# alibaba/graph-gpt

Hardware: AMD Instinct MI355X
Metric: graph-tokens/sec (un-padded Eulerian tokens, whole job) + SMTP loss, PCQM4M-v2 base pre-train (higher is better)
Workload: dtype bf16; 1 GPU; pcqm4m-v2-pretrain-base; model=base d768/L12/H12 (122.1M params), per_gpu_batch=256, global_batch=256, seq_len=32, stacked_feat=13, vocab=756, parallelism=dp1, step=fwd+bwd+allreduce+clip+AdamW, reproducible_mode=True

## Files before the change

graph-gpt_amd/_lib.py:

```python
from __future__ import annotations

import contextlib
import ctypes as C
import os

HERE = os.path.dirname(os.path.abspath(__file__))
LIB_PATH = os.environ.get("GGET_LIB_PATH") or os.path.join(HERE, "lib", "libgget_hip.so")

i32, i64, u64, f32, vp, cp = C.c_int32, C.c_int64, C.c_uint64, C.c_float, C.c_void_p, C.c_char_p


class GgetConfig(C.Structure):
    _fields_ = [(n, i32) for n in ("kind", "vocab_size", "hidden_size", "intermediate_size", "num_layers", "num_heads",
                                   "stacked_feat", "next_n_token", "gated_agg", "causal", "max_position", "num_labels",
                                   "score_bias", "pad_token_id")] + \
               [("rms_eps", f32), ("rope_theta", f32), ("layer_scale_init", f32), ("max_tokens", i32), ("max_batch", i32),
                ("path_pdrop", f32), ("mlp_pdrop", f32), ("head_mlp_layers", i32), ("head_mlp", i32 * 4), ("embed_dim", i32)]


class GgetSizes(C.Structure):
    _fields_ = [(n, u64) for n in ("n_params", "param_bf16_bytes", "master_bytes", "adam_bytes", "grad_bf16_bytes",
                                   "workspace_bytes")]


# ... 64 lines not shown
    "gget_debug_set": (i32, [i32, i32]),
    "gget_debug_get": (i32, [i32, C.POINTER(i32)]),
    "gget_debug_occupy": (i32, [vp, u64, i32, i32, i32, vp]),
    "gget_op_gemm_grouped": (i32, [i32, i32, vp, vp, vp, vp, vp, vp, vp, vp, vp, vp]),
    "gget_op_rmsnorm_fwd": (i32, [vp, vp, vp, vp, i32, i32, f32, vp]),
    "gget_op_rmsnorm_bwd": (i32, [vp, vp, vp, vp, vp, vp, vp, i32, i32, vp]),
    "gget_op_embed_fwd": (i32, [vp, vp, vp, vp, i32, i32, i32, i32, vp]),
    "gget_op_embed_bwd": (i32, [vp, vp, vp, vp, vp, vp, i32, i32, i32, i32, i32, i32, vp]),
    "gget_op_qkv_rope": (i32, [vp, vp, vp, vp, vp, vp, i32, i32, i32, vp]),
    "gget_op_smtp2d": (i32, [vp, i32, vp, i32, vp, vp, i32, i32, i32, f32, f32, f32, i32, i32, C.c_uint32, vp]),
    "gget_op_token_sample": (i32, [vp, i32, i32, i32, i32, f32, f32, i32, f32, C.c_uint32, vp, vp, vp]),
    "gget_op_unmask_origin": (i32, [vp, vp, i32, i32, f32, C.c_uint32, i32, vp]),
    "gget_op_unmask_origin_rows": (i32, [vp, vp, i32, i32, vp, C.c_uint32, i32, vp]),
    "gget_op_unmask_ranked": (i32, [vp, vp, vp, i32, i32, i32, vp, i32, vp, vp]),
    "gget_op_gen_plan": (i32, [vp, i32, i32, i32, vp, i32, vp, vp, vp, vp]),
    "gget_op_gen_acc": (i32, [vp, vp, vp, i32, i32, i32, vp, vp]),
    "gget_op_token_confidence": (i32, [vp, i32, i32, i32, i32, vp, vp, vp]),
    "gget_op_smtp_rows": (i32, [vp, vp, vp, vp, vp, i32, i32, i32, C.c_double, C.c_double, C.c_double, C.c_uint32, vp]),
    "gget_op_rope": (i32, [vp, vp, vp, vp, i32, i32, i32, i32, vp]),
    "gget_op_attn_fwd": (i32, [vp, vp, vp, vp, i32, i32, i32, i32, vp, vp, vp, f32, C.c_uint32, vp]),
    "gget_op_attn_bwd": (i32, [vp, vp, vp, vp, vp, vp, vp, i32, i32, i32, i32, vp, vp, vp, f32, C.c_uint32, vp]),
    "gget_op_copy_from_host": (i32, [vp, vp, C.c_uint64, vp]),
    "gget_op_attn_fwd_varlen": (i32, [vp, vp, vp, vp, vp, i32, i32, i32, i32, vp, vp, vp, i32, f32, C.c_uint32, vp]),
    "gget_op_attn_bwd_varlen": (i32, [vp, vp, vp, vp, vp, vp, vp, vp, i32, i32, i32, i32, vp, vp, vp, i32, f32, C.c_uint32, vp]),
    "gget_op_attn_oproj_fwd": (i32, [vp, vp, vp, vp, vp, vp, vp, vp, vp, vp, vp, i32, i32, i32, i32, f32, f32, C.c_uint32, vp, vp]),
    "gget_op_pack_wo": (i32, [vp, C.c_uint64, vp, vp, i32, i32, vp]),
    "gget_op_attn_oproj_bwd": (i32, [vp, vp, vp, vp, vp, vp, vp, i32, C.c_uint64, vp, vp, vp, vp, vp, vp, i32, i32, i32, i32, vp, vp, vp, f32,
                                      C.c_uint32, i32, vp, vp, vp]),
    "gget_op_attn_fwd_ranges": (i32, [vp, vp, vp, vp, vp, i32, i32, i32, i32, f32, C.c_uint32, vp]),
    "gget_op_attn_bwd_ranges": (i32, [vp, vp, vp, vp, vp, vp, vp, vp, i32, i32, i32, i32, f32, C.c_uint32, vp]),
    "gget_op_ranges_from_mask3d": (i32, [vp, vp, vp, i32, i32, vp]),
    "gget_op_attn_bwd_fused": (i32, [vp, vp, vp, vp, vp, vp, vp, vp, vp, vp, i32, i32, i32, i32, f32, C.c_uint32, vp]),
    "gget_set_dropout": (i32, [vp, f32, f32, C.c_uint32]),
    "gget_set_auc": (i32, [vp, i32, C.c_uint32]),
    "gget_set_token_count": (i32, [vp, C.c_int64]),
    "gget_set_option": (i32, [vp, i32, i32]),
    "gget_set_dp_menu": (i32, [vp, i32, i32]),
    "gget_varlen_status": (i32, [vp, vp, vp]),
    "gget_position_status": (i32, [vp, vp, vp]),
    "gget_deferred_status": (i32, [vp, vp, vp]),
    "gget_set_focal_gamma": (i32, [vp, f32]),
    "gget_set_stack_method": (i32, [vp, i32]),
    "gget_set_rope_range": (i32, [vp, f32]),
    "gget_set_raw_embeds": (i32, [vp, vp, i32]),
    "gget_debug_probe": (i32, [vp, i32, C.POINTER(f32)]),
    "gget_debug_gemm_probe": (i32, [i32, C.POINTER(C.c_double), C.POINTER(C.c_double), C.POINTER(i32), C.POINTER(i32)]),
    "gget_set_dropout_ex": (i32, [vp, f32, f32, f32]),
    "gget_op_gateup_geglu": (i32, [vp, vp, vp, vp, i32, i32, i32, vp]),
    "gget_op_down_dgrad_geglu": (i32, [vp, vp, vp, vp, vp, i32, i32, i32, vp]),
    "gget_op_geglu_fwd": (i32, [vp, vp, i32, i32, vp]),
    "gget_op_geglu_bwd": (i32, [vp, vp, vp, i32, i32, vp]),
    "gget_op_ce_fwd_bwd": (i32, [vp, i32, vp, vp, vp, i32, i32, vp, vp, f32, i32, vp]),
    "gget_op_rmsnorm_bwd_copies": (i32, [vp, vp, vp, vp, vp, vp, vp, i32, i32, i32, u64, vp]),
    "gget_op_rmsnorm_dw": (i32, [vp, vp, vp, vp, i32, i32, i32, u64, vp]),
    "gget_op_ls_rmsnorm_fwd": (i32, [vp, vp, vp, vp, vp, vp, vp, i32, i32, f32, vp]),
    "gget_op_accum_layout": (i32, [i32, C.POINTER(i32), C.POINTER(u64)]),
    "gget_op_rmsnorm_bwd_ls": (i32, [vp, vp, vp, vp, vp, vp, vp, vp, vp, vp, vp, i32, i32, vp]),
    "gget_op_rope_table": (i32, [vp, vp, i32, f32, vp]),
    "gget_op_rope_range_table": (i32, [vp, vp, vp, vp, i32, i32, f32, f32, vp]),
    "gget_op_clamp_positions": (i32, [vp, vp, vp, i64, i32, vp]),
    "gget_op_embed_long_ratio": (i32, [vp, vp, i32, i32, i32, i32, vp]),
    "gget_op_ce_full": (i32, [vp, i32, vp, vp, vp, i32, vp, i32, i32, vp, vp, f32, i32, vp, f32, vp, i32, vp]),
    "gget_op_score_fwd": (i32, [vp, vp, vp, vp, vp, vp, i32, i32, i32, vp]),
    "gget_op_score_bwd": (i32, [vp, vp, vp, vp, vp, vp, vp, i32, i32, i32, vp]),
    "gget_op_tok_score_fwd": (i32, [vp, vp, vp, vp, i32, i32, i32, vp]),
    "gget_op_tok_intra_fwd": (i32, [vp, vp, vp, vp, i32, i32, i32, vp]),
    "gget_op_tok_intra_bwd": (i32, [vp, vp, vp, vp, vp, vp, i32, i32, i32, vp]),
    "gget_set_cls_idx": (i32, [vp, vp]),
    "gget_op_tok_ce": (i32, [vp, vp, vp, vp, vp, i32, i32, vp, i32, vp]),
    "gget_op_tok_score_bwd": (i32, [vp, vp, vp, vp, vp, vp, vp, i32, i32, i32, vp]),
    "gget_op_task_loss": (i32, [vp, vp, vp, i32, i32, i32, vp, vp, vp]),
    "gget_op_auc_loss": (i32, [vp, vp, i32, i32, i32, C.c_uint32, vp, vp, vp, vp]),
    "gget_op_pool_rows": (i32, [vp, vp, vp, i32, i32, vp]),
    "gget_op_scatter_rows_f32": (i32, [vp, vp, vp, i32, i32, vp]),
    "gget_op_head_linear_fwd": (i32, [vp, vp, vp, vp, vp, vp, i32, i32, i32, i32, vp]),
    "gget_op_head_linear_bwd": (i32, [vp, vp, vp, vp, vp, vp, vp, i32, i32, i32, i32, vp]),
    "gget_op_lengths": (i32, [vp, vp, i32, i32, vp, vp, i32, i32, vp]),
    "gget_op_sum_lengths": (i32, [vp, i32, vp, vp]),
    "gget_op_varlen_plan": (i32, [vp, i32, i32, vp, vp, vp, vp, vp, vp, vp, vp, vp, vp, i32, i32, i32, i32, i32, vp, vp]),
    "gget_op_rows_to_grid": (i32, [vp, vp, vp, i64, i32, vp]),
    "gget_op_head_compact_ws_bytes": (u64, [i32]),
    "gget_op_head_compact": (i32, [vp, i32, i32, vp, vp, vp, vp, vp, vp, vp, vp, vp, vp, vp]),
    "gget_op_head_slot_sort": (i32, [vp, vp, vp, vp, vp, vp, vp, vp, vp, vp, i32, i32, i64, i32, vp]),
    "gget_op_head_cell_sum": (i32, [vp, vp, vp, vp, vp, vp, i32, i32, i32, vp]),
    "gget_op_gather_rows": (i32, [vp, vp, vp, vp, i32, i32, i32, vp]),
    "gget_op_gather_rows_remap": (i32, [vp, vp, vp, vp, vp, i32, i32, i32, vp, vp]),
    "gget_op_sample_mask_wgt": (i32, [vp, vp, i32, i32, vp]),
    "gget_op_raw_blend": (i32, [vp, vp, i32, i32, vp, vp, vp, i32, i32, vp, i32, vp]),
    "gget_op_raw_tok_grad": (i32, [vp, vp, vp, i32, i32, vp]),
    "gget_op_gemm_indexed": (i32, [i32, vp, vp, vp, i32, i32, i32, i32, i32, i32, vp, vp, vp, i32, vp, vp]),
    "gget_op_rank_metrics_workspace": (C.c_size_t, [i32, i32]),
    "gget_op_rank_metrics": (i32, [vp, i32, vp, i32, i32, i32, vp, vp, vp, vp, vp, vp, C.c_size_t, vp]),
    "gget_op_link_hits_workspace": (C.c_size_t, [i32]),
    "gget_op_link_hits": (i32, [vp, vp, i32, i64, vp, vp, vp, vp, vp, vp, C.c_size_t, vp]),
    "gget_op_link_mrr_workspace": (C.c_size_t, [i32]),
    "gget_op_link_mrr": (i32, [vp, vp, vp, i32, i32, i32, vp, vp, vp, vp, vp, vp, vp, vp, C.c_size_t, vp]),
    "gget_op_cluster_metrics": (i32, [vp, i32, vp, vp, i32, i32, i32, vp, vp, vp, vp]),
}
CLUSTER_MAX_C = 2048

GEMM_NT, GEMM_NN, GEMM_TN = 0, 1, 2
OPT_NORM_FROM_BACKWARD = 1
OPT_SKIP_NONFINITE_STEP = 2
SHARD_CHUNK = 4096
SHARD_PARAMS, SHARD_MASTER, SHARD_ADAM_M, SHARD_ADAM_V, SHARD_SLOTS, SHARD_EMA = 0, 1, 2, 3, 4, 5
TOKENS_AUTO = -2
EPI_NONE, EPI_RESIDUAL, EPI_ATOMIC_F32, EPI_SLAB_F32 = 0, 1, 2, 3

KEY_GEMM_VARIANT, KEY_GEMM_LDS_HEADROOM, KEY_GEMM_SPLIT_LAST, KEY_DETERMINISTIC, KEY_GEMM_STAGGER = 1, 2, 3, 4, 5
KEY_GEMM_ABLATE, KEY_HEAD_DENSE, KEY_HEAD_TILE, KEY_ATTN_OPROJ_OFF, KEY_LS_NORM_BWD_WIDE = 7, 8, 9, 10, 11
KEY_RMS_WIDE, KEY_CE_PARTS, KEY_GEMM_CU_RESERVE, KEY_OCCUPY_FAT, KEY_LINK_GRID, KEY_CE_GENERIC = 13, 14, 15, 16, 18, 19
KEY_EMBED_SORTED = 20
MENU_KEYS = (1, 2, 3, 4, 5, 7, 8, 9, 10, 11, 13, 14, 15, 16, 18, 19, 20)
GEMM_NO_KSPLIT_ND, GEMM_NO_KSPLIT_WGRAD, GEMM_NO_192_ROWS, GEMM_NO_SPLIT_LAST, GEMM_KSPLIT_128_ONLY, GEMM_ONE_BLOCK_PER_CU = 1, 2, 4, 8, 16, 32
GEMM_KSPLIT_DMA8, GEMM_AREA_RULE = 128, 512


def debug_get(key: int) -> int:
    v = i32()
    check(load().gget_debug_get(int(key), C.byref(v)))
    return int(v.value)


@contextlib.contextmanager
def debug_menu(keys):
    saved = {k: debug_get(k) for k in keys}
    try:
        for k, v in keys.items():
            check(load().gget_debug_set(int(k), int(v)))
        yield
    finally:
        for k, v in saved.items():
            check(load().gget_debug_set(k, v))


def gemm_grouped(lib, mode, problems, stream):
    n = len(problems)
    PA, IA = vp * n, i32 * n
    ptr = lambda k: PA(*[p[k].data_ptr() for p in problems])
    num = lambda k: IA(*[int(p[k]) for p in problems])
    return lib.gget_op_gemm_grouped(mode, n, ptr(0), ptr(1), ptr(2), num(3), num(4), num(5), num(6), num(7), num(8), stream)
PROBLEM_SINGLE_LABEL, PROBLEM_REGRESSION_L1, PROBLEM_REGRESSION_MSE, PROBLEM_MULTI_LABEL, PROBLEM_AUC = 0, 1, 2, 3, 4
PROBLEM_TOKEN_CE_INTRA = 6
PROBLEM_TOKEN_CE = 5

_lib = None


class GgetError(RuntimeError):
    pass


def load(path: str = LIB_PATH):
    global _lib
    if _lib is not None:
        return _lib
    import torch
    if not os.path.exists(path):
        raise GgetError(f"{path} is missing: build it with `python graph-gpt_amd/build.py` "
                        "(or __graft_entry__.build()); this engine has no CPU fallback")
    lib = C.CDLL(path)
    for name, (res, args) in SIGNATURES.items():
        fn = getattr(lib, name)
        fn.restype = res
        fn.argtypes = args
    _lib = lib
    return lib


def check(rc: int):
    if rc != 0:
        raise GgetError(f"gget error {rc}: {load().gget_last_error().decode()}")
```

graph-gpt_amd/csrc/engine.hip:

```cpp
#include <dlfcn.h>
#include <stdarg.h>
#include <stdio.h>
#include <string.h>

#include <algorithm>
#include <chrono>
#include <string>
#include <functional>
#include <vector>

#include "common.h"
#include "gemm.h"
#include "kernels.h"
#include <rccl/rccl.h>

static thread_local char g_err[512] = "";
void gget_set_error(const char* fmt, ...) {
  va_list ap;
  va_start(ap, fmt);
  vsnprintf(g_err, sizeof(g_err), fmt, ap);
  va_end(ap);
}
extern "C" const char* gget_last_error(void) { return g_err; }
extern "C" int gget_version(void) { return 101; }
// ... 77 lines not shown
  add_param(pl, "model.embed_tokens.weight", V, d, -1, true, &pl.emb, &pl.emb32);
  if (pl.has_gate) add_param(pl, "stacked_feat_agg.weight", F, d, -1, true, &pl.gate, &pl.gate32);
  if (c.embed_dim > 0) {
    add_param(pl, "embed_layernorm.weight", c.embed_dim, 0, -1, true, &pl.raw_ln, &pl.raw_ln32);
    if (c.kind == GGET_KIND_PRETRAIN) add_param(pl, "emb_mask_token", c.embed_dim, 0, -1, true, &pl.raw_tok, &pl.raw_tok32);
    add_param(pl, "embed_proj.weight", d, c.embed_dim, -1, false, &pl.raw_proj, nullptr);
  }
  pl.layers.resize(L);
  for (int i = 0; i < L; ++i) {
    LayerOff& lo = pl.layers[i];
    const std::string p = "model.layers." + std::to_string(i) + ".";
    add_param(pl, p + "input_layernorm.weight", d, 0, i, true, &lo.ln1, &lo.ln1_32);
    add_param(pl, p + "self_attn.q_proj.weight", d, d, i, false, &lo.wqkv, nullptr);
    add_param(pl, p + "self_attn.k_proj.weight", d, d, i, false, nullptr, nullptr);
    add_param(pl, p + "self_attn.v_proj.weight", d, d, i, false, nullptr, nullptr);
    add_param(pl, p + "self_attn.o_proj.weight", d, d, i, false, &lo.wo, nullptr);
    if (pl.has_ls) add_param(pl, p + "lambda_1", d, 0, i, true, &lo.lam1, &lo.lam1_32);
    add_param(pl, p + "post_attention_layernorm.weight", d, 0, i, true, &lo.ln2, &lo.ln2_32);
    add_param(pl, p + "mlp.gate_proj.weight", ff, d, i, false, &lo.wgu, nullptr);
    add_param(pl, p + "mlp.up_proj.weight", ff, d, i, false, nullptr, nullptr);
    add_param(pl, p + "mlp.down_proj.weight", d, ff, i, false, &lo.wdown, nullptr);
    if (pl.has_ls) add_param(pl, p + "lambda_2", d, 0, i, true, &lo.lam2, &lo.lam2_32);
  }
  add_param(pl, "model.norm.weight", d, 0, (int)L, true, &pl.normf, &pl.normf32);
  if (c.kind == GGET_KIND_PRETRAIN) {
    if (pl.has_ntp) add_param(pl, "n_token_proj.weight", (int64_t)c.next_n_token * d, d, (int)L, false, &pl.ntp, nullptr);
    add_param(pl, "lm_head.weight", V, d, (int)L, false, &pl.lm, nullptr);
    const int64_t Vp = (int64_t)align_up((uint64_t)V, 64);
    pl.lm_pad_off = pl.n_params;
    pl.lm_pad_count = (uint64_t)(Vp - V) * d;
    pl.n_params += align_up(pl.lm_pad_count, 128);
  } else {
    if (c.head_mlp_layers > 0) {
      pl.n_lin = c.head_mlp_layers + 1;
      pl.head_dim[0] = (int)d;
      for (int i = 0; i < c.head_mlp_layers; ++i) pl.head_dim[i + 1] = c.head_mlp[i];
      pl.head_dim[pl.n_lin] = c.num_labels;
      for (int i = 0; i < pl.n_lin; ++i) {
        const std::string p = "score.mlp_modules." + std::to_string(i) + ".";
        add_param(pl, p + "weight", pl.head_dim[i + 1], pl.head_dim[i], (int)L, true, &pl.head_w[i], &pl.head_w32[i]);
        if (c.score_bias) add_param(pl, p + "bias", pl.head_dim[i + 1], 0, (int)L, true, &pl.head_b[i], &pl.head_b32[i]);
      }
    } else {
      add_param(pl, "score.weight", c.num_labels, d, (int)L, true, &pl.score, &pl.score32);
      if (c.score_bias) add_param(pl, "score.bias", c.num_labels, 0, (int)L, true, &pl.sbias, &pl.sbias32);
    }
  }
  return pl;
}

struct Bump {
  uint64_t off = 0;
  uint64_t take(uint64_t bytes) {
    const uint64_t o = off;
    off += align_up(bytes, 256);
    return o;
  }
};

struct LayerWs {
  uint64_t rstd1, xn1, qkv, lse, attn, araw, xmid, rstd2, xn2, gu, h, mraw;
};

struct Ws {
  uint64_t key_len, pool_row, cos_tab, sin_tab, key_lo, key_hi;
  std::vector<uint64_t> xres;
  std::vector<LayerWs> lw;
  uint64_t rstd_f, hidden;
  uint64_t dxa, dxb, dxc, dxn, dqkv, dattn, dgu, dh, delta, dq_acc, dscaled, dscaled2;
  uint64_t scratch32, loss_sum, loss_part, sqnorm, counts, segs, emb_sort, emb_cnt, emb_slab, wg32, lm_slab;
  uint64_t sq_chunks, sq_tiles;
  uint64_t cnt, hc_tot, m_off, l_off, row_idx, sel_src, sel_label, sel_tok, Hm, Pp, Hl, logits, dlogits, dHl, dP, dHm;
  uint64_t ss_tok, ss_cell, ss_l, ss_pos, ss_tile, ss_state, ss_total;
  uint64_t tlogits, tdlogits, pooled_h, auc_lists;
  uint64_t raw_x, raw_xn, raw_rstd, raw_dxn, raw_dx, raw_flag;
  uint64_t rr_cos, rr_sin, rr_ids;
  uint64_t tok_stat;
  uint64_t intra_rs, intra_cls;
  uint64_t long_wgt;
  uint64_t vl_cu, vl_rowb, vl_pos, vl_ids, vl_pad2c, vl_c2p, vl_status;
  uint64_t vl_long;
  uint64_t wo_pack = 0, wot_pack = 0;
  uint64_t pos_safe;
  uint64_t sk_ws;
  uint64_t head_x[6] = {0}, head_a[5] = {0}, head_d[2] = {0};
  uint64_t total;
};

Ws make_ws(const gget_config_t& c, const Plan& pl) {
  Ws w;
  Bump b;
  const uint64_t T = c.max_tokens, d = c.hidden_size, ff = c.intermediate_size, H = c.num_heads, L = c.num_layers;
  const uint64_t Bm = c.max_batch;
  w.key_len = b.take(Bm * 4);
  w.key_lo = b.take(T * 4);
  w.key_hi = b.take(T * 4);
  w.pool_row = b.take(Bm * 4);
  w.cos_tab = b.take((uint64_t)c.max_position * 32 * 4);
  w.sin_tab = b.take((uint64_t)c.max_position * 32 * 4);
  w.xres.resize(L + 1);
  for (uint64_t i = 0; i <= L; ++i) w.xres[i] = b.take(T * d * 2);
  w.lw.resize(L);
  for (uint64_t i = 0; i < L; ++i) {
    LayerWs& l = w.lw[i];
    l.rstd1 = b.take(T * 4);
    l.xn1 = b.take(T * d * 2);
    l.qkv = b.take(T * 3 * d * 2);
    l.lse = b.take(T * H * 4);
    l.attn = b.take(T * d * 2);
    l.araw = pl.has_res ? b.take(T * d * 2) : 0;
    l.xmid = b.take(T * d * 2);
    l.rstd2 = b.take(T * 4);
    l.xn2 = b.take(T * d * 2);
    l.gu = b.take(T * 2 * ff * 2);
    l.h = b.take(T * ff * 2);
    l.mraw = pl.has_res ? b.take(T * d * 2) : 0;
  }
  w.rstd_f = b.take(T * 4);
  w.hidden = b.take(T * d * 2);
  w.dxa = b.take(T * d * 2);
  w.dxb = b.take(T * d * 2);
  w.dxc = b.take(T * d * 2);
  w.dxn = b.take(T * d * 2);
  w.dqkv = b.take(T * 3 * d * 2);
  w.dattn = b.take(T * d * 2);
  w.dgu = b.take(T * 2 * ff * 2);
  w.dh = b.take(T * ff * 2);
  w.delta = b.take(T * H * 4);
  {
    const uint64_t Smax = c.max_tokens / (c.max_batch > 0 ? c.max_batch : 1);
    w.dq_acc = Smax >= 256 ? b.take(((Smax + 255) / 256) * T * d * 2) : 0;
  }
  w.dscaled = pl.has_res ? b.take(T * d * 2) : 0;
  w.dscaled2 = pl.has_res ? b.take(T * d * 2) : 0;
  w.scratch32 = b.take(pl.n_scratch32 * 4);
  w.loss_sum = b.take(256);
  w.loss_part = b.take(2048 * sizeof(float));
  w.sqnorm = b.take(k_grad_sqnorm_ws_bytes());
  w.sq_chunks = b.take(1024 * sizeof(GgetSqChunk));
  w.sq_tiles = b.take((uint64_t)c.num_layers * kSqTilesPerLayer * sizeof(float));
  w.counts = b.take(256);
  w.segs = b.take((uint64_t)pl.params.size() * sizeof(GgetSegment));
  w.wg32 = b.take(kWgSplit * 4 * d * d * 4);
  w.long_wgt = b.take((uint64_t)c.max_batch * 4);
  w.vl_cu = b.take((Bm + 1) * 4);
  w.vl_long = b.take((3 * Bm + 1) * 4);
  w.vl_rowb = b.take(T * 4);
  w.vl_pos = b.take(T * 8);
  w.vl_ids = b.take(T * (uint64_t)c.stacked_feat * 8);
  w.vl_pad2c = b.take(T * 4);
  w.vl_c2p = b.take(T * 4);
  if (d % 64 == 0 && !pl.has_res) {
    w.wo_pack = b.take((uint64_t)c.num_layers * d * d * 2);
    w.wot_pack = b.take((uint64_t)c.num_layers * d * d * 2);
  }
  w.vl_status = b.take(256);
  w.pos_safe = b.take(T * 8);
  w.sk_ws = b.take(gget_gemm_streamk_bytes());
  if (c.embed_dim > 0) {
    const uint64_t e = c.embed_dim;
    w.raw_x = b.take(T * e * 2); w.raw_xn = b.take(T * e * 2); w.raw_rstd = b.take(T * 4);
    w.raw_dxn = b.take(T * e * 2); w.raw_dx = b.take(T * e * 2); w.raw_flag = b.take(T * 4);
  }
  w.rr_cos = b.take(T * 32 * 4);
  w.rr_sin = b.take(T * 32 * 4);
  w.rr_ids = b.take(T * 8);
  w.emb_sort = b.take(k_embed_bwd_ws_elems(T * (uint64_t)c.stacked_feat, (uint64_t)c.vocab_size) * 4);
  w.emb_cnt = k_embed_dense_ok(c.vocab_size, pl.has_gate) ? b.take(T * align_up(c.vocab_size, 64) * 2) : 0;
  w.emb_slab = k_embed_dense_ok(c.vocab_size, pl.has_gate) ? b.take((uint64_t)kEmbDenseSplit * c.vocab_size * d * 4) : 0;
  if (c.kind == GGET_KIND_PRETRAIN) {
    const uint64_t n = c.next_n_token, Vp = align_up(c.vocab_size, 64);
    w.cnt = b.take(T * 4);
    w.hc_tot = b.take(k_head_compact_ws_bytes((int)T));
    w.m_off = b.take(T * 4);
    w.l_off = b.take(T * 4);
    w.row_idx = b.take(T * 4);
    w.sel_src = b.take(T * n * 4);
    w.sel_label = b.take(T * n * 4);
    w.sel_tok = b.take(T * n * 4);
    w.Hm = b.take(T * d * 2);
    w.dHm = b.take(T * d * 2);
    if (n > 1) {
      const uint64_t cap_p = T * n + n * 256;
      w.ss_tok = b.take(cap_p * 4);
      w.ss_cell = b.take(cap_p * 4);
      w.ss_l = b.take(cap_p * 4);
      w.ss_pos = b.take(T * n * 4);
      w.ss_tile = b.take((cap_p / 128 + 1) * 4);
      w.ss_state = b.take(512);
      w.ss_total = b.take(256);
      w.Pp = b.take(cap_p * d * 2);
      w.Hl = b.take(T * n * d * 2);
      w.dHl = b.take(T * n * d * 2);
      w.dP = b.take(T * n * d * 2);
    } else {
      w.Pp = w.Hl = w.Hm;
      w.dHl = w.dP = w.dHm;
    }
    w.lm_slab = b.take((uint64_t)kLmSplit * c.vocab_size * d * 4);
    w.logits = b.take(T * n * Vp * 2);
    w.dlogits = b.take(T * n * Vp * 2);
  } else {
    w.tlogits = b.take(std::max(Bm, T) * c.num_labels * 4);
    w.tdlogits = b.take(std::max(Bm, T) * c.num_labels * 4);
    w.tok_stat = b.take(256);
    w.intra_rs = b.take((Bm + 1) * 4);
    w.intra_cls = b.take(Bm * 8);
    w.auc_lists = b.take(Bm * 2 * 4);
    w.pooled_h = b.take(Bm * d * 2);
    if (pl.n_lin > 0) {
      uint64_t dmax = 0;
      for (int i = 0; i <= pl.n_lin; ++i) dmax = std::max<uint64_t>(dmax, (uint64_t)pl.head_dim[i]);
      w.head_x[0] = w.pooled_h;
      for (int i = 1; i <= pl.n_lin; ++i) w.head_x[i] = b.take(Bm * pl.head_dim[i] * 2);
      for (int i = 0; i < pl.n_lin; ++i) w.head_a[i] = b.take(Bm * pl.head_dim[i] * 2);
      w.head_d[0] = b.take(Bm * dmax * 4);
      w.head_d[1] = b.take(Bm * dmax * 4);
    }
  }
  w.total = b.off;
  return w;
}

int check_cfg(const gget_config_t* c) {
  GGET_REQUIRE(c != nullptr, "null config");
  GGET_REQUIRE(c->hidden_size > 0 && c->hidden_size % 64 == 0, "hidden_size must be a positive multiple of 64");
  GGET_REQUIRE(c->num_heads * 64 == c->hidden_size, "num_heads*64 must equal hidden_size (head_dim is 64)");
  GGET_REQUIRE(c->intermediate_size > 0 && c->intermediate_size % 64 == 0, "intermediate_size must be a multiple of 64");
  GGET_REQUIRE(c->hidden_size <= 2048, "hidden_size > 2048 not supported by the norm kernels");
  GGET_REQUIRE(c->vocab_size > 1 && c->num_layers >= 1 && c->stacked_feat >= 1, "bad vocab/layers/stacked_feat");
  GGET_REQUIRE(c->kind == GGET_KIND_PRETRAIN || c->kind == GGET_KIND_TASK, "bad kind");
  GGET_REQUIRE(c->max_tokens > 0 && c->max_batch > 0 && c->max_position > 0, "bad capacities");
  if (c->kind == GGET_KIND_PRETRAIN) GGET_REQUIRE(c->next_n_token >= 1, "next_n_token must be >= 1");
  else GGET_REQUIRE(c->num_labels >= 1, "num_labels must be >= 1");
  GGET_REQUIRE(c->embed_dim >= 0 && c->embed_dim % 64 == 0 && c->embed_dim <= 2048, "embed_dim must be 0 or a multiple of 64 up to 2048");
  GGET_REQUIRE(c->head_mlp_layers >= 0 && c->head_mlp_layers <= 4, "the MLP score head holds at most 4 hidden layers");
  for (int i = 0; i < c->head_mlp_layers; ++i) GGET_REQUIRE(c->head_mlp[i] > 0, "bad MLP head width");
  return 0;
}

}

static int bucket_of(int layer, int L) { return layer == L ? 0 : layer < 0 ? L + 1 : L - layer; }

static std::vector<std::pair<uint64_t, uint64_t>> bucket_ranges(const gget_config_t& cfg, const Plan& plan) {
  const int L = cfg.num_layers;
  std::vector<std::pair<uint64_t, uint64_t>> r(L + 2, {UINT64_MAX, 0});
  for (const ParamRec& p : plan.params) {
    auto& b = r[bucket_of(p.layer, L)];
    b.first = std::min(b.first, p.off);
    b.second = std::max(b.second, p.off + align_up(p.count, 128));
  }
  if (plan.lm_pad_count) {
    auto& b = r[bucket_of(L, L)];
    b.second = std::max(b.second, plan.lm_pad_off + align_up(plan.lm_pad_count, 128));
  }
// ... 35 lines not shown
    GGET_HIP_CHECK(hipMalloc(&tab, b_it + b_ch + b_cs + b_gs));
    items = reinterpret_cast<const GgetSqChunk*>(tab);
    chunks = items + it.size();
    chunk_slot = reinterpret_cast<const int32_t*>(chunks + ch.size());
    slot_of = chunk_slot + ch_slot.size();
    auto put = [](const void* dst, const void* src, size_t bytes) {
      return bytes ? hipMemcpy(const_cast<void*>(dst), src, bytes, hipMemcpyHostToDevice) : hipSuccess;
    };
    GGET_HIP_CHECK(put(items, it.data(), b_it));
    GGET_HIP_CHECK(put(chunks, ch.data(), b_ch));
    GGET_HIP_CHECK(put(chunk_slot, ch_slot.data(), b_cs));
    GGET_HIP_CHECK(put(slot_of, global_slot.data(), b_gs));
    nitems = (int)it.size();
    nchunks = (int)ch.size();
    nglobal = (int)global_slot.size();
    return 0;
  }
};

struct gget_engine {
  gget_config_t cfg;
  Plan plan;
  Ws ws;
  bf16_t* P;
  float* master;
  float* am;
  float* av;
  float* ema = nullptr;
  float ema_decay_next = -1.f;
  bf16_t* G;
  float* grad_acc = nullptr;
  int grad_acc_count = 0;
  bool grad_from_acc() const { return grad_acc != nullptr && grad_acc_count > 0; }
  const void* grad_src() const { return grad_from_acc() ? (const void*)grad_acc : (const void*)G; }
  unsigned char* W;
  const float* cos_tab;
  const float* sin_tab;
  std::vector<std::pair<uint64_t, uint64_t>> bucket_range;
  std::vector<std::pair<int, int>> bucket_segs;
  int B = 0, S = 0, T = 0, TP = 0;
  bool varlen = false;
  bool wo_packed = false;
  int tc = 0;
  long tc_next = -1;
  bool opt_norm_from_backward = false;
  bool opt_skip_nonfinite = false;
  bool step_needs_norm(float max_grad_norm, const float* gnorm_dev) const { return max_grad_norm > 0.f || gnorm_dev != nullptr || opt_skip_nonfinite; }
  int sq_layers = 0;
  int n_sq_chunks = 0;
  bool emb_cnt_cleared = false;
  bool head_sorted_fwd = false;
  bool tc_from_caller = false;
  int32_t* host_word = nullptr;
  int32_t* host_word_dev = nullptr;
  const int64_t* pos_rows = nullptr;
  const int32_t* row_base() const { return varlen ? wsp<int32_t>(ws.vl_cu) : nullptr; }
  const int32_t* long_list() const { return varlen ? wsp<int32_t>(ws.vl_long) : nullptr; }
  const int64_t* ids = nullptr;
  const int64_t* pos = nullptr;
  const float* sample_wgt = nullptr;
  bool have_labels = false;
  int problem = 0;
  int auc_num_neg = 1;
  const int64_t* cls_idx_next = nullptr;
  float focal_gamma = 0.f;
  bool stack_long = false;
  float rope_range = 0.f;
  const float* raw_next = nullptr;
  bool raw_first_label_only = false;
  bool ls2_done = false;
  bool raw_used = false;
  const float* cos_cur = nullptr;
  const float* sin_cur = nullptr;
  const int64_t* pos_cur = nullptr;
  bool probe = false;
  std::vector<hipEvent_t> probe_ev[2];
  hipEvent_t probe_event(int which, int idx) {
    auto& v = probe_ev[which];
    while ((int)v.size() <= idx) { hipEvent_t e; if (hipEventCreate(&e) != hipSuccess) return nullptr; v.push_back(e); }
    return v[idx];
  }
  std::function<int(hipStream_t)> presync_work;
  bool presync_done = false;
  hipEvent_t count_event = nullptr;
  unsigned auc_seed = 0;
  bool fwd_valid = false;
  float attn_drop_p = 0.f;
  float path_drop_p = 0.f;
  unsigned attn_drop_seed = 0;
  float embed_drop_p = 0.f;
  float mlp_drop_p = 0.f;
  float head_drop_p = 0.f;
  ElemDropArg head_drop() const { return elem_drop(head_drop_p, attn_drop_seed ^ 0x2545F491u); }
  static ElemDropArg elem_drop(float p, unsigned seed, const int32_t* rows = nullptr) {
    if (p <= 0.f) return ElemDropArg{0, 1.f, 0, nullptr};
    return ElemDropArg{(unsigned)(p * 16777216.0f), 1.0f / (1.0f - p), seed, rows};
  }
  const int32_t* drop_rows() const { return varlen ? wsp<int32_t>(ws.vl_c2p) : nullptr; }
  ElemDropArg embed_drop() const { return elem_drop(embed_drop_p, attn_drop_seed ^ 0x5BD1E995u, drop_rows()); }
  ElemDropArg mlp_drop(int layer) const { return elem_drop(mlp_drop_p, attn_drop_seed + 0x7F4A7C15u * (unsigned)(layer + 1), drop_rows()); }
  PathDropArg path_drop(int layer, int which) const {
    const int L = cfg.num_layers;
    const float rate = (path_drop_p > 0.f && L > 1) ? path_drop_p * (float)layer / (float)(L - 1) : 0.f;
    return PathDropArg{rate, attn_drop_seed ^ (0xD6E8FEB8u * (unsigned)(layer * 2 + which + 1)), S, varlen ? wsp<int32_t>(ws.vl_rowb) : nullptr};
  }
  bf16_t* dx_cur = nullptr;
  bool packed = false;
  bool defer_convert = false;
  void* comm = nullptr;
  bool comm_loopback = false;
  int comm_rank = 0, comm_world = 1;
  int dp_reserve_cus = 0;
  bool dp_lds_headroom = false;
  float* comm_f32 = nullptr;
  uint64_t comm_f32_elems = 0;
  int shard_world = 0, shard_rank = 0;
  int shard_slots = 0;
  std::vector<ShardBucket> shard_plan;
  OptWork shard_work;
  int frozen = -1;
  std::vector<std::pair<uint64_t, uint64_t>> train_ranges;
  OptWork frozen_work;
  const OptWork* opt_work(bool sharded) const { return sharded ? &shard_work : frozen >= 0 ? &frozen_work : nullptr; }
  bool truncated() const { return frozen >= 0 && !plan.has_gate && cfg.embed_dim == 0; }
  int first_trainable_layer() const { return frozen < 0 ? 0 : std::min(frozen, cfg.num_layers); }
  std::pair<uint64_t, uint64_t> bucket_train_range(int bucket) const {
    const uint64_t lo = bucket_range[bucket].first, hi = bucket_range[bucket].second;
    if (frozen < 0) return {lo, hi - lo};
    for (const auto& r : train_ranges) {
      const uint64_t a = std::max(lo, r.first), b = std::min(hi, r.first + r.second);
      if (a < b) return {a, b - a};
    }
    return {lo, 0};
  }
  const int32_t* klo() const { return packed ? wsp<int32_t>(ws.key_lo) : nullptr; }
  const int32_t* khi() const { return packed ? wsp<int32_t>(ws.key_hi) : nullptr; }

  template <typename Tp>
  Tp* wsp(uint64_t off) const { return reinterpret_cast<Tp*>(W + off); }
  int bucket_of_layer(int layer) const { return bucket_of(layer, cfg.num_layers); }
};

struct CallScope {
  LaunchMenu m;
  explicit CallScope(gget_engine* h) : m(g_menu) {
    if (h->dp_reserve_cus > 0) {
      m.gemm_cu_reserve = h->dp_reserve_cus;
      m.gemm_lds_headroom = 1;
      m.rms_wide = 0;
    } else if (h->dp_lds_headroom) {
      m.gemm_lds_headroom = 2;
    }
    t_call_menu = &m;
    gget_gemm_streamk_workspace(h->W + h->ws.sk_ws);
  }
  ~CallScope() {
    gget_gemm_streamk_workspace(nullptr);
    t_call_menu = nullptr;
  }
};

extern "C" int gget_query_sizes(const gget_config_t* cfg, gget_sizes_t* out) {
  if (int e = check_cfg(cfg)) return e;
  GGET_REQUIRE(out != nullptr, "null out");
  Plan pl = make_plan(*cfg);
  Ws w = make_ws(*cfg, pl);
// ... 136 lines not shown
  GGET_REQUIRE(embed_p >= 0.f && embed_p < 1.f && mlp_p >= 0.f && mlp_p < 1.f && head_p >= 0.f && head_p < 1.f,
               "dropout probabilities must be in [0, 1)");
  h->head_drop_p = head_p;
  GGET_REQUIRE(mlp_p == 0.f || h->cfg.mlp_pdrop > 0.f, "MLP dropout needs a handle created with config.mlp_pdrop > 0");
  h->embed_drop_p = embed_p;
  h->mlp_drop_p = mlp_p;
  return 0;
}

extern "C" int gget_set_raw_embeds(gget_handle_t h, const float* raw_embeds_dev, int first_label_only) {
  GGET_REQUIRE(h != nullptr, "null handle");
  GGET_REQUIRE(h->cfg.embed_dim > 0 || raw_embeds_dev == nullptr, "the handle was created with embed_dim = 0");
  h->raw_next = raw_embeds_dev;
  h->raw_first_label_only = first_label_only != 0;
  return 0;
}

extern "C" int gget_set_rope_range(gget_handle_t h, float rope_range) {
  GGET_REQUIRE(h != nullptr, "null handle");
  GGET_REQUIRE(rope_range >= 0.f, "rope_range must be >= 0");
  h->rope_range = rope_range;
  return 0;
}

extern "C" int gget_set_stack_method(gget_handle_t h, int stack_long) {
  GGET_REQUIRE(h != nullptr, "null handle");
  h->stack_long = stack_long != 0;
  return 0;
}

extern "C" int gget_set_focal_gamma(gget_handle_t h, float gamma) {
  GGET_REQUIRE(h != nullptr, "null handle");
  GGET_REQUIRE(gamma >= 0.f, "focal_gamma must be >= 0");
  h->focal_gamma = gamma;
  return 0;
}

extern "C" int gget_set_auc(gget_handle_t h, int num_neg, uint32_t seed) {
  GGET_REQUIRE(h != nullptr, "null handle");
  GGET_REQUIRE(num_neg >= 1, "num_neg must be >= 1");
  h->auc_num_neg = num_neg;
  h->auc_seed = seed;
  return 0;
}

extern "C" int gget_set_cls_idx(gget_handle_t h, const int64_t* cls_idx_dev) {
  GGET_REQUIRE(h != nullptr, "null handle");
  h->cls_idx_next = cls_idx_dev;
  return 0;
}

extern "C" int gget_set_token_count(gget_handle_t h, int64_t n_real_tokens) {
  GGET_REQUIRE(h != nullptr, "null handle");
  h->tc_next = n_real_tokens > 0 ? (long)n_real_tokens : (n_real_tokens == GGET_TOKENS_AUTO ? (long)GGET_TOKENS_AUTO : -1);
  return 0;
}

extern "C" int gget_set_option(gget_handle_t h, int option, int value) {
  GGET_REQUIRE(h != nullptr, "null handle");
  switch (option) {
    case GGET_OPT_NORM_FROM_BACKWARD: h->opt_norm_from_backward = value != 0; return 0;
    case GGET_OPT_SKIP_NONFINITE_STEP: h->opt_skip_nonfinite = value != 0; return 0;
  }
  gget_set_error("set_option: unknown option %d", option);
  return 2;
}

extern "C" int gget_set_dp_menu(gget_handle_t h, int reserve_cus, int lds_headroom) {
  GGET_REQUIRE(h != nullptr, "null handle");
  GGET_REQUIRE(reserve_cus >= 0, "set_dp_menu: reserve_cus %d < 0", reserve_cus);
  h->dp_reserve_cus = reserve_cus;
  h->dp_lds_headroom = lds_headroom != 0;
  return 0;
}

extern "C" int gget_deferred_status(gget_handle_t h, int32_t out[2], void* stream) {
  GGET_REQUIRE(h && out, "null argument");
  int32_t* st = h->wsp<int32_t>(h->ws.vl_status);
  GGET_HIP_CHECK(hipMemcpyAsync(&out[0], st + 1, 4, hipMemcpyDeviceToHost, (hipStream_t)stream));
  GGET_HIP_CHECK(hipMemcpyAsync(&out[1], st + 2, 4, hipMemcpyDeviceToHost, (hipStream_t)stream));
  int32_t cls_clamped = 0;
  GGET_HIP_CHECK(hipMemcpyAsync(&cls_clamped, st + 4, 4, hipMemcpyDeviceToHost, (hipStream_t)stream));
  GGET_HIP_CHECK(hipMemsetAsync(st + 1, 0, 8, (hipStream_t)stream));
  GGET_HIP_CHECK(hipMemsetAsync(st + 4, 0, 4, (hipStream_t)stream));
  GGET_HIP_CHECK(hipStreamSynchronize((hipStream_t)stream));
  if (cls_clamped) out[0] |= 2;
  return 0;
}

extern "C" int gget_position_status(gget_handle_t h, int32_t* clamped_out, void* stream) {
  GGET_REQUIRE(h && clamped_out, "null argument");
  int32_t* flag = h->wsp<int32_t>(h->ws.vl_status) + 1;
  GGET_HIP_CHECK(hipMemcpyAsync(clamped_out, flag, 4, hipMemcpyDeviceToHost, (hipStream_t)stream));
  GGET_HIP_CHECK(hipMemsetAsync(flag, 0, 4, (hipStream_t)stream));
  GGET_HIP_CHECK(hipStreamSynchronize((hipStream_t)stream));
  return 0;
}

extern "C" int gget_varlen_status(gget_handle_t h, int32_t out[3], void* stream) {
  GGET_REQUIRE(h && out, "null argument");
  out[0] = h->varlen ? 1 : 0;
  out[1] = h->T;
  out[2] = 0;
  if (h->varlen) {
    GGET_HIP_CHECK(hipMemcpyAsync(&out[2], h->wsp<int32_t>(h->ws.vl_status), 4, hipMemcpyDeviceToHost, (hipStream_t)stream));
    GGET_HIP_CHECK(hipStreamSynchronize((hipStream_t)stream));
  }
  return 0;
}

extern "C" int gget_set_dropout(gget_handle_t h, float attention_p, float path_p, uint32_t seed) {
  GGET_REQUIRE(h, "null handle");
  GGET_REQUIRE(attention_p >= 0.f && attention_p < 1.f && path_p >= 0.f && path_p < 1.f, "dropout probability out of range");
  GGET_REQUIRE(path_p == 0.f || h->plan.has_res, "path dropout needs a handle created with config.path_pdrop > 0");
  h->attn_drop_p = attention_p;
  h->path_drop_p = path_p;
  h->attn_drop_seed = seed;
  return 0;
}

extern "C" int gget_sync_params(gget_handle_t h, void* stream) {
  GGET_REQUIRE(h && h->master, "sync_params needs the fp32 master arena");
  h->wo_packed = false;
  return k_f32_to_bf16(h->master, h->P, h->plan.n_params, (hipStream_t)stream);
}

namespace {

int gemm_nt(const void* A, const void* Bw, void* C, const void* R, int M, int N, int K, int lda, int ldb, int ldc,
            const int* m_dev, hipStream_t st) {
  return gget_gemm_single(GGET_GEMM_NT, R ? GGET_EPI_RESIDUAL : GGET_EPI_NONE, A, Bw, C, R, M, N, K, lda, ldb, ldc, m_dev,
                          nullptr, 1, st);
}
int gemm_nn(const void* A, const void* Bw, void* C, int M, int N, int K, int lda, int ldb, int ldc, const int* m_dev,
            hipStream_t st, const int* c_rows = nullptr) {
  return gget_gemm_single(GGET_GEMM_NN, GGET_EPI_NONE, A, Bw, C, nullptr, M, N, K, lda, ldb, ldc, m_dev, nullptr, 1, st, false, c_rows);
}
inline int head_tile_rows(int d) { return menu().head_tile == 128 ? 128 : ((d % 256) == 0 ? 256 : 128); }
bool head_scatter_fused() { return !menu().no_head_scatter_fusion; }
bool head_sorted() { return menu().head_sorted && !menu().head_dense && head_scatter_fused(); }

bool geglu_fusable(int d, int ff) { return !menu().no_geglu_fusion && ff % 128 == 0 && d % 64 == 0; }
int gateup_geglu(const bf16_t* x, const bf16_t* wgu, bf16_t* gu, bf16_t* hh, int T, int d, int ff, hipStream_t st) {
  if (!geglu_fusable(d, ff)) {
    if (int e = gemm_nt(x, wgu, gu, nullptr, T, 2 * ff, d, d, d, 2 * ff, nullptr, st)) return e;
    return k_geglu_fwd(gu, hh, T, ff, st);
  }
  GemmGroup g;
  memset(&g, 0, sizeof(g));
  g.count = 1;
  GemmProblem& p = g.p[0];
  p.A = x; p.B = wgu; p.C = gu; p.C2 = hh;
  p.M = T; p.N = 2 * ff; p.K = d; p.lda = d; p.ldb = d; p.ldc = 2 * ff; p.ldc2 = ff; p.ff = ff;
  return gget_gemm_launch(GGET_GEMM_NT, GGET_EPI_GEGLU_FWD, g, 1, st);
}
int down_dgrad_geglu(const bf16_t* dy, const bf16_t* wdown, const bf16_t* gu, bf16_t* dgu, bf16_t* dh_scratch, int T, int d, int ff,
                     hipStream_t st) {
  if (!geglu_fusable(d, ff)) {
    if (int e = gemm_nn(dy, wdown, dh_scratch, T, ff, d, d, ff, ff, nullptr, st)) return e;
    return k_geglu_bwd(gu, dh_scratch, dgu, T, ff, st);
  }
  GemmGroup g;
  memset(&g, 0, sizeof(g));
  g.count = 1;
  GemmProblem& p = g.p[0];
  p.A = dy; p.B = wdown; p.C = dgu; p.G = gu;
  p.M = T; p.N = ff; p.K = d; p.lda = d; p.ldb = ff; p.ldc = 2 * ff; p.ldg = 2 * ff; p.ff = ff;
  return gget_gemm_launch(GGET_GEMM_NN, GGET_EPI_GEGLU_BWD, g, 1, st);
}
// ... 435 lines not shown
    bf16_t* mraw = h->wsp<bf16_t>(lw.mraw);
    const bf16_t* lam1 = h->plan.has_ls ? h->P + lo.lam1 : nullptr;
    const bf16_t* lam2 = h->plan.has_ls ? h->P + lo.lam2 : nullptr;
    const PathDrop pd1 = h->path_drop(i, 0), pd2 = h->path_drop(i, 1);
    const int g = (int)std::min<long>(4096, ((long)T * (d / 8) + 255) / 256);
    if (int e = gemm_nt(attn, h->P + lo.wo, araw, nullptr, T, d, d, d, d, d, nullptr, st)) return e;
    const bool fused = ls_norm_fused();
    if (fused) {
      if (int e = ls_rmsnorm_fwd(x_in, araw, lam1, xmid, h->P + lo.ln2, xn2, h->wsp<float>(lw.rstd2), T, d, c.rms_eps, pd1,
                                 ElemDropArg{0, 1.f, 0}, st))
        return e;
    } else {
      hipLaunchKernelGGL(ls_fwd_kernel, dim3(g), dim3(256), 0, st, x_in, araw, lam1, xmid, (long)T, d, pd1, ElemDropArg{0, 1.f, 0});
      if (int e = k_rmsnorm_fwd(xmid, h->P + lo.ln2, xn2, h->wsp<float>(lw.rstd2), T, d, c.rms_eps, st)) return e;
    }
    if (int e = gateup_geglu(xn2, h->P + lo.wgu, gu, hh, T, d, ff, st)) return e;
    const ElemDropArg md = h->mlp_drop(i);
    if (int e = k_elem_dropout(hh, T, ff, GGET_DROP_STREAM_MLP_ACT, md, st)) return e;
    if (int e = gemm_nt(hh, h->P + lo.wdown, mraw, nullptr, T, d, ff, ff, ff, d, nullptr, st)) return e;
    if (fused) {
      const bool last = i + 1 == c.num_layers;
      const bf16_t* nw = last ? h->P + h->plan.normf : h->P + h->plan.layers[i + 1].ln1;
      bf16_t* nxn = last ? h->wsp<bf16_t>(h->ws.hidden) : h->wsp<bf16_t>(h->ws.lw[i + 1].xn1);
      float* nrs = last ? h->wsp<float>(h->ws.rstd_f) : h->wsp<float>(h->ws.lw[i + 1].rstd1);
      return ls_rmsnorm_fwd(xmid, mraw, lam2, x_out, nw, nxn, nrs, T, d, c.rms_eps, pd2, md, st);
    }
    hipLaunchKernelGGL(ls_fwd_kernel, dim3(g), dim3(256), 0, st, xmid, mraw, lam2, x_out, (long)T, d, pd2, md);
    GGET_LAUNCH_CHECK();
    return 0;
  }
  if (int e = gemm_nt(attn, h->P + lo.wo, xmid, x_in, T, d, d, d, d, d, nullptr, st)) return e;
  if (int e = k_rmsnorm_fwd(xmid, h->P + lo.ln2, xn2, h->wsp<float>(lw.rstd2), T, d, c.rms_eps, st)) return e;
  if (h->probe) GGET_HIP_CHECK(hipEventRecord(h->probe_event(1, 2 * i), st));
  if (int e = gateup_geglu(xn2, h->P + lo.wgu, gu, hh, T, d, ff, st)) return e;
  if (h->probe) GGET_HIP_CHECK(hipEventRecord(h->probe_event(1, 2 * i + 1), st));
  if (int e = gemm_nt(hh, h->P + lo.wdown, x_out, xmid, T, d, ff, ff, ff, d, nullptr, st)) return e;
  return 0;
}

bool varlen_enabled() { return !menu().no_varlen; }
int backbone_forward(gget_engine* h, long tc_hint, const int64_t* ids, int ldF, const int64_t* mask, const int64_t* pos, int B, int S,
                     hipStream_t st, bool mask_is_3d = false, const int64_t* labels = nullptr, bool allow_varlen = true) {
  const gget_config_t& c = h->cfg;
  GGET_REQUIRE(B > 0 && S > 0, "empty batch");
  GGET_REQUIRE((long)B * S <= c.max_tokens && B <= c.max_batch, "batch %dx%d exceeds capacity (%d tokens, %d rows)", B, S,
               c.max_tokens, c.max_batch);
  GGET_REQUIRE(S <= c.max_position, "sequence length %d exceeds max_position %d", S, c.max_position);
  h->B = B; h->S = S; h->T = h->TP = B * S;
  if (pos && !(h->rope_range > 0.f)) {
    if (int e = k_clamp_positions(pos, h->wsp<int64_t>(h->ws.pos_safe), h->wsp<int32_t>(h->ws.vl_status) + 1, (long)B * S, c.max_position, st))
      return e;
    pos = h->wsp<int64_t>(h->ws.pos_safe);
  }
  h->ids = ids; h->pos = pos;
  h->cos_cur = h->cos_tab; h->sin_cur = h->sin_tab; h->pos_cur = pos;
  h->varlen = false;
  h->tc_from_caller = false;
  h->tc = B * S;
  const int d = c.hidden_size;
  h->packed = mask_is_3d;
  auto pack_o_weights = [&]() -> int {
    h->wo_packed = false;
    const bool may_varlen = allow_varlen && varlen_enabled() && (tc_hint > 0 || tc_hint == GGET_TOKENS_AUTO) && mask != nullptr;
    const int ncu = gget_gemm_num_cu() > 0 ? gget_gemm_num_cu() : 256;
    const int rounds = (B + ncu - 1) / ncu;
    const bool rounds_ok = B <= ncu || (long)B * 100 >= (long)rounds * ncu * 85;
    if (!h->plan.has_res && !mask_is_3d && (S <= 32 || (S <= 64 && may_varlen)) && rounds_ok && h->ws.wo_pack && c.num_layers > 0) {
      const size_t stride = c.num_layers > 1 ? h->plan.layers[1].wo - h->plan.layers[0].wo : 0;
      bool regular = true;
      for (int i = 0; i < c.num_layers; ++i) regular = regular && h->plan.layers[i].wo == h->plan.layers[0].wo + (size_t)i * stride;
      if (regular) {
        if (int e = k_pack_wo(h->P + h->plan.layers[0].wo, stride, h->wsp<bf16_t>(h->ws.wo_pack), h->wsp<bf16_t>(h->ws.wot_pack), d, c.num_layers, st))
          return e;
        h->wo_packed = true;
      }
    }
    return 0;
  };
  bool early_done = false;
  auto early_work = [&]() -> int {
    if (early_done) return 0;
    early_done = true;
    if (int e = pack_o_weights()) return e;
    if (h->presync_work) {
      if (int e = h->presync_work(st)) return e;
      h->presync_done = true;
    }
    return 0;
  };
  if (mask_is_3d) {
    GGET_REQUIRE(mask != nullptr && c.kind == GGET_KIND_PRETRAIN, "a 3-D (packed) attention mask needs the pre-train model and a mask");
    if (int e = k_ranges_from_mask3d(mask, h->wsp<int32_t>(h->ws.key_lo), h->wsp<int32_t>(h->ws.key_hi), B, S, st)) return e;
  } else if (int e = k_lengths(mask, c.kind == GGET_KIND_TASK ? ids : nullptr, ldF, c.pad_token_id,
                               h->wsp<int32_t>(h->ws.key_len),
                               c.kind == GGET_KIND_TASK ? h->wsp<int32_t>(h->ws.pool_row) : nullptr, B, S, st)) {
    return e;
  }
  if (allow_varlen && varlen_enabled() && (tc_hint > 0 || tc_hint == GGET_TOKENS_AUTO) && !mask_is_3d && mask != nullptr) {
    long tc = tc_hint;
    if (tc_hint == GGET_TOKENS_AUTO) {
      int32_t* dst = h->wsp<int32_t>(h->ws.vl_status) + 3;
      if (!h->host_word) {
        GGET_HIP_CHECK(hipHostMalloc(reinterpret_cast<void**>(&h->host_word), 64, hipHostMallocMapped | hipHostMallocCoherent));
        GGET_HIP_CHECK(hipHostGetDevicePointer(reinterpret_cast<void**>(&h->host_word_dev), h->host_word, 0));
      }
      const bool count_copy = menu().count_copy != 0;
      constexpr int32_t kNoCount = INT32_MIN;
      if (!count_copy) __atomic_store_n(h->host_word, kNoCount, __ATOMIC_RELEASE);
      if (int e = k_sum_lengths(h->wsp<int32_t>(h->ws.key_len), B, dst, st, count_copy ? nullptr : h->host_word_dev)) return e;
      if (count_copy) {
        GGET_HIP_CHECK(hipMemcpyAsync(h->host_word, dst, 4, hipMemcpyDeviceToHost, st));
        if (!h->count_event) GGET_HIP_CHECK(hipEventCreateWithFlags(&h->count_event, hipEventDisableTiming));
        GGET_HIP_CHECK(hipEventRecord(h->count_event, st));
      }
      if (int e = early_work()) return e;
      if (count_copy) {
        GGET_HIP_CHECK(hipEventSynchronize(h->count_event));
        tc = *h->host_word;
      } else {
        int32_t v = kNoCount;
        const auto t0 = std::chrono::steady_clock::now();
        for (long spin = 0; (v = __atomic_load_n(h->host_word, __ATOMIC_ACQUIRE)) == kNoCount; ++spin) {
#if defined(__x86_64__)
          __builtin_ia32_pause();
#endif
          if ((spin & 1023) == 1023 && std::chrono::steady_clock::now() - t0 > std::chrono::seconds(2)) {
            GGET_HIP_CHECK(hipStreamSynchronize(st));
            v = __atomic_load_n(h->host_word, __ATOMIC_ACQUIRE);
            GGET_REQUIRE(v != kNoCount, "the token count never arrived from the device");
            break;
          }
        }
        tc = v;
      }
    }
    const long t_rows = (tc + 63) / 64 * 64;
    if (tc > 0 && t_rows < (long)B * S) {
      h->varlen = true;
      h->tc_from_caller = tc_hint > 0;
      h->tc = (int)tc;
      h->T = (int)t_rows;
    }
  }
  if (int e = early_work()) return e;
  if (h->rope_range > 0.f && pos) {
    if (int e = k_rope_range_table(pos, h->wsp<float>(h->ws.rr_cos), h->wsp<float>(h->ws.rr_sin), h->wsp<int64_t>(h->ws.rr_ids), B, S,
                                   h->rope_range, c.rope_theta > 0.f ? c.rope_theta : 10000.0f, st))
      return e;
    h->cos_cur = h->wsp<float>(h->ws.rr_cos); h->sin_cur = h->wsp<float>(h->ws.rr_sin); h->pos_cur = h->wsp<int64_t>(h->ws.rr_ids);
  }
  h->pos_rows = h->pos_cur;
  if (h->varlen) {
    const Ws& w = h->ws;
    if (int e = k_varlen_plan(ids, ldF, c.stacked_feat, h->pos_cur, h->wsp<int32_t>(w.key_len),
                              c.kind == GGET_KIND_TASK ? h->wsp<int32_t>(w.pool_row) : nullptr, h->wsp<int32_t>(w.vl_cu),
                              h->wsp<int64_t>(w.vl_ids), h->wsp<int64_t>(w.vl_pos), h->wsp<int32_t>(w.vl_rowb), h->wsp<int32_t>(w.vl_pad2c),
                              h->wsp<int32_t>(w.vl_c2p), h->wsp<int32_t>(w.vl_status), B, S, h->tc, h->T, c.pad_token_id, st,
                              h->wsp<int32_t>(w.vl_long)))
      return e;
    h->ids = ids = h->wsp<int64_t>(w.vl_ids);
    ldF = c.stacked_feat;
    h->pos_rows = h->wsp<int64_t>(w.vl_pos);
  }
  if (int e = k_embed_fwd(ids, h->P + h->plan.emb, h->plan.has_gate ? h->P + h->plan.gate : nullptr,
                          h->wsp<bf16_t>(h->ws.xres[0]), h->T, c.stacked_feat, ldF, d, st, h->embed_drop()))
    return e;
  if (h->stack_long)
    if (int e = k_embed_long_ratio(ids, h->wsp<bf16_t>(h->ws.xres[0]), h->T, c.stacked_feat, ldF, d, st)) return e;
  h->raw_used = false;
  if (c.embed_dim > 0) {
    GGET_REQUIRE(h->raw_next != nullptr, "this model was built with embed_dim > 0: hand the raw embeddings over with gget_set_raw_embeds");
    const Ws& w = h->ws;
    const int e_ = c.embed_dim;
    const bool blend = c.kind == GGET_KIND_PRETRAIN && labels != nullptr;
    if (int e = k_raw_blend(h->raw_next, blend ? labels : nullptr, c.next_n_token, h->raw_first_label_only,
                            blend ? h->P + h->plan.raw_tok : nullptr, h->wsp<bf16_t>(w.raw_x), h->wsp<int32_t>(w.raw_flag), h->T, e_, st,
                            h->varlen ? h->wsp<int32_t>(w.vl_c2p) : nullptr, B * S))
      return e;
    if (int e = k_rmsnorm_fwd(h->wsp<bf16_t>(w.raw_x), h->P + h->plan.raw_ln, h->wsp<bf16_t>(w.raw_xn), h->wsp<float>(w.raw_rstd), h->T, e_,
                              c.rms_eps, st))
      return e;
    if (int e = k_elem_dropout(h->wsp<bf16_t>(w.raw_xn), h->T, e_, GGET_DROP_STREAM_RAW, h->embed_drop(), st)) return e;
    bf16_t* x0 = h->wsp<bf16_t>(w.xres[0]);
    if (int e = gemm_nt(h->wsp<bf16_t>(w.raw_xn), h->P + h->plan.raw_proj, x0, x0, h->T, d, e_, e_, e_, d, nullptr, st)) return e;
    h->raw_used = true;
    h->raw_next = nullptr;
  }
  for (int i = 0; i < c.num_layers; ++i)
    if (int e = layer_forward(h, i, st)) return e;
  if (h->plan.has_res && ls_norm_fused()) return 0;
  return k_rmsnorm_fwd(h->wsp<bf16_t>(h->ws.xres[c.num_layers]), h->P + h->plan.normf, h->wsp<bf16_t>(h->ws.hidden),
                       h->wsp<float>(h->ws.rstd_f), h->T, d, c.rms_eps, st);
}

}

static int forward_pretrain_impl(gget_handle_t h, const int64_t* input_ids_dev, const int64_t* attention_mask_dev,
                                 bool mask_is_3d, const int64_t* labels_dev, const float* sample_wgt_dev,
                                 const int64_t* position_ids_dev, int B, int S, float* loss_dev, void* stream) {
  GGET_REQUIRE(h != nullptr, "null argument");
  const long tc_hint = h->tc_next;
  h->tc_next = -1;
  GGET_REQUIRE(input_ids_dev, "null argument");
  GGET_REQUIRE(h->cfg.kind == GGET_KIND_PRETRAIN, "handle was not created as a pre-train model");
  hipStream_t st = (hipStream_t)stream;
  const gget_config_t& c = h->cfg;
  CallScope scope(h);
  h->fwd_valid = false;
  const Ws& w = h->ws;
  const int d = c.hidden_size, n = c.next_n_token, V = c.vocab_size;
  const int Vp = (int)align_up(V, 64);
  int32_t* counts = h->wsp<int32_t>(w.counts);
  const bool sorted_head = h->plan.has_ntp && head_sorted() && d % 192 == 0 && n <= 32;
  auto head_compact = [&](hipStream_t s_) -> int {
    return k_head_compact(labels_dev, B * S, n, h->wsp<int32_t>(w.cnt), h->wsp<int32_t>(w.m_off), h->wsp<int32_t>(w.l_off), counts,
                          h->wsp<int32_t>(w.row_idx), h->wsp<int32_t>(w.sel_src), h->wsp<int32_t>(w.sel_label), h->wsp<int32_t>(w.sel_tok),
                          h->wsp<int32_t>(w.hc_tot), sorted_head ? h->wsp<int32_t>(w.ss_state) : nullptr, s_);
  };
  h->presync_work = head_compact;
  h->presync_done = false;
  const int rc_bb = backbone_forward(h, tc_hint, input_ids_dev, c.stacked_feat, attention_mask_dev, position_ids_dev, B, S, st, mask_is_3d, labels_dev);
  h->presync_work = nullptr;
  if (rc_bb) {
    if (sorted_head && h->presync_done)
      (void)hipMemsetAsync(h->wsp<int32_t>(w.ss_state), 0, 512, st);
    return rc_bb;
  }
  const int T = h->TP;
  if (!h->presync_done)
    if (int e = head_compact(st)) return e;
  if (h->varlen) {
    if (int e = k_gather_rows_remap(h->wsp<bf16_t>(w.hidden), h->wsp<int32_t>(w.row_idx), counts, h->wsp<int32_t>(w.vl_pad2c),
                                    h->wsp<bf16_t>(w.Hm), T, d, h->T > h->tc ? h->tc : 0, labels_dev ? h->wsp<int32_t>(w.vl_status) : nullptr, st))
      return e;
  } else if (int e = k_gather_rows(h->wsp<bf16_t>(w.hidden), h->wsp<int32_t>(w.row_idx), counts, h->wsp<bf16_t>(w.Hm), T, d, 0, st))
    return e;
  h->head_sorted_fwd = false;
  if (sorted_head) {
    if (int e = k_head_slot_sort(h->wsp<int32_t>(w.sel_src), h->wsp<int32_t>(w.row_idx), counts + 1, h->wsp<int32_t>(w.ss_state),
                                 h->wsp<int32_t>(w.ss_tok), h->wsp<int32_t>(w.ss_cell), h->wsp<int32_t>(w.ss_l), h->wsp<int32_t>(w.ss_pos),
                                 h->wsp<int32_t>(w.ss_tile), h->wsp<int32_t>(w.ss_total), T * n, n, (long)d * d, head_tile_rows(d), st))
      return e;
    GemmGroup g;
    memset(&g, 0, sizeof(g));
    g.count = 1;
    GemmProblem& p = g.p[0];
    p.A = h->wsp<bf16_t>(w.hidden); p.B = h->P + h->plan.ntp; p.C = h->wsp<bf16_t>(w.Hl);
    p.M = T * n + n * 256; p.N = d; p.K = d; p.lda = d; p.ldb = d; p.ldc = d;
    p.m_dev = h->wsp<int32_t>(w.ss_total);
    p.a_rows = h->wsp<int32_t>(w.ss_tok); p.b_tile_off = h->wsp<int32_t>(w.ss_tile); p.c_rows = h->wsp<int32_t>(w.ss_l);
    p.b_tile_rows = head_tile_rows(d);
    if (int e = gget_gemm_launch(GGET_GEMM_NT, GGET_EPI_NONE, g, 1, st)) return e;
    h->head_sorted_fwd = true;
  } else if (h->plan.has_ntp) {
    if (int e = gemm_nt(h->wsp<bf16_t>(w.Hm), h->P + h->plan.ntp, h->wsp<bf16_t>(w.Pp), nullptr, T, n * d, d, d, d, n * d,
                        counts, st))
      return e;
    if (int e = k_gather_rows(h->wsp<bf16_t>(w.Pp), h->wsp<int32_t>(w.sel_src), counts + 1, h->wsp<bf16_t>(w.Hl), T * n, d, 0,
                              st))
      return e;
  }
  if (int e = gemm_nt(h->wsp<bf16_t>(w.Hl), h->P + h->plan.lm, h->wsp<bf16_t>(w.logits), nullptr, T * n, V, d, d, d, Vp,
                      counts + 1, st))
    return e;
  h->have_labels = labels_dev != nullptr;
  if (h->stack_long && labels_dev) {
    if (int e = k_sample_mask_wgt(labels_dev, h->wsp<float>(w.long_wgt), B, S * n, st)) return e;
    sample_wgt_dev = h->wsp<float>(w.long_wgt);
  }
  h->sample_wgt = sample_wgt_dev;
  if (labels_dev) {
    const int mean_rows = sample_wgt_dev == nullptr;
    const float base = 1.0f / (float)((long)B * S * n);
    if (int e = k_ce_fwd_bwd(h->wsp<bf16_t>(w.logits), Vp, h->wsp<int32_t>(w.sel_label), h->wsp<int32_t>(w.sel_tok),
                             sample_wgt_dev, S, counts + 1, T * n, V, h->wsp<float>(w.loss_sum), h->wsp<bf16_t>(w.dlogits),
                             base, mean_rows, loss_dev, st, mean_rows ? h->focal_gamma : 0.f, h->wsp<float>(w.loss_part), 2048))
      return e;
    if (h->varlen && h->tc_from_caller && loss_dev)
      if (int e = k_poison_loss(h->wsp<int32_t>(w.vl_status), loss_dev, st)) return e;
  }
  h->fwd_valid = true;
  return 0;
}

extern "C" int gget_forward_pretrain(gget_handle_t h, const int64_t* input_ids_dev, const int64_t* attention_mask_dev,
                                     const int64_t* labels_dev, const float* sample_wgt_dev,
                                     const int64_t* position_ids_dev, int B, int S, float* loss_dev, void* stream) {
  return forward_pretrain_impl(h, input_ids_dev, attention_mask_dev, false, labels_dev, sample_wgt_dev, position_ids_dev, B, S,
                               loss_dev, stream);
}

extern "C" int gget_forward_pretrain_packed(gget_handle_t h, const int64_t* input_ids_dev, const int64_t* attention_mask3d_dev,
                                            const int64_t* labels_dev, const float* sample_wgt_dev,
                                            const int64_t* position_ids_dev, int B, int S, float* loss_dev, void* stream) {
  GGET_REQUIRE(attention_mask3d_dev != nullptr, "the packed forward needs the [B,S,S] mask");
  return forward_pretrain_impl(h, input_ids_dev, attention_mask3d_dev, true, labels_dev, sample_wgt_dev, position_ids_dev, B, S,
                               loss_dev, stream);
}

extern "C" int gget_forward_task(gget_handle_t h, const int64_t* input_ids_dev, const int64_t* attention_mask_dev,
                                 const int64_t* position_ids_dev, const void* task_labels_dev, const float* sample_wgt_dev,
                                 int problem_type, int B, int S, float* loss_dev, float* task_logits_dev,
                                 void* task_hidden_dev, void* stream) {
  GGET_REQUIRE(h != nullptr, "null argument");
  const long tc_hint = h->tc_next;
  h->tc_next = -1;
  const int64_t* cls_idx_dev = h->cls_idx_next;
  h->cls_idx_next = nullptr;
  GGET_REQUIRE(input_ids_dev, "null argument");
  GGET_REQUIRE(h->cfg.kind == GGET_KIND_TASK, "handle was not created as a task model");
  const bool tok = problem_type == GGET_PROBLEM_TOKEN_CE || problem_type == GGET_PROBLEM_TOKEN_CE_INTRA;
  GGET_REQUIRE(problem_type != GGET_PROBLEM_TOKEN_CE_INTRA || cls_idx_dev, "the intra-instance token head needs cls_idx (gget_set_cls_idx)");
  hipStream_t st = (hipStream_t)stream;
  const gget_config_t& c = h->cfg;
  CallScope scope(h);
  h->fwd_valid = false;
  if (int e = backbone_forward(h, tc_hint, input_ids_dev, c.stacked_feat, attention_mask_dev, position_ids_dev, B, S, st, false, nullptr))
    return e;
  const Ws& w = h->ws;
  const int d = c.hidden_size, C = c.num_labels;
  float* lg = h->wsp<float>(w.tlogits);
  GGET_REQUIRE(!tok || h->plan.n_lin == 0, "the token-level head is the Linear `score` (no MLP head)");
  if (h->plan.n_lin > 0) {
    const Plan& pl = h->plan;
    if (int e = k_pool_rows(h->wsp<bf16_t>(w.hidden), h->wsp<int32_t>(w.pool_row), h->wsp<bf16_t>(w.pooled_h), B, d, st)) return e;
// ... 1142 lines not shown
  return k_tok_intra_bwd(dl, stat, hidden, row_start, cls_idx, dhidden, B, C, d, (hipStream_t)stream);
}
extern "C" int gget_op_tok_ce(const float* logits, const int64_t* labels, float* dl, float* stat, float* loss_out, int T, int C,
                              const int32_t* rows_map, int n_logical, void* stream) {
  GGET_REQUIRE(logits && labels && dl && stat && loss_out && T >= 0 && C > 0, "tok_ce: null argument or empty shape");
  return k_tok_ce(logits, labels, dl, stat, loss_out, T, C, (hipStream_t)stream, rows_map, n_logical);
}
extern "C" int gget_op_tok_score_bwd(const float* dl, const float* stat, const void* hidden, const void* w, float* dw, float* dbias,
                                     void* dhidden, int T, int C, int d, void* stream) {
  GGET_REQUIRE(dl && stat && hidden && w && dw && dhidden && T >= 0 && C > 0, "tok_score_bwd: null argument or empty shape");
  GGET_REQUIRE(d % 64 == 0 && d > 0 && d <= 1024, "token-level head: d=%d unsupported", d);
  return k_tok_score_bwd(dl, stat, hidden, w, dw, dbias, dhidden, T, C, d, (hipStream_t)stream);
}
extern "C" int gget_op_task_loss(const float* logits, const void* labels, const float* sample_wgt, int problem, int B, int C,
                                 float* loss_out, float* dlogits, void* stream) {
  GGET_REQUIRE(logits && labels && loss_out && dlogits && B > 0 && C > 0, "task_loss: null argument or empty shape");
  GGET_REQUIRE(problem == GGET_PROBLEM_SINGLE_LABEL || problem == GGET_PROBLEM_REGRESSION_L1 || problem == GGET_PROBLEM_REGRESSION_MSE ||
                   problem == GGET_PROBLEM_MULTI_LABEL,
               "task_loss: problem type %d has a kernel of its own", problem);
  return k_task_loss(logits, labels, sample_wgt, problem, B, C, loss_out, dlogits, (hipStream_t)stream);
}
extern "C" int gget_op_auc_loss(const float* logits, const int64_t* labels, int B, int C, int num_neg, uint32_t seed, float* loss_out,
                                float* dlogits, int32_t* lists, void* stream) {
  GGET_REQUIRE(logits && labels && loss_out && dlogits && lists, "auc_loss: null argument");
  return k_auc_loss(logits, labels, B, C, num_neg, seed, loss_out, dlogits, lists, (hipStream_t)stream);
}
extern "C" int gget_op_pool_rows(const void* hidden, const int32_t* pool_row, void* out, int B, int d, void* stream) {
  GGET_REQUIRE(hidden && pool_row && out && B > 0 && d > 0, "pool_rows: null argument or empty shape");
  return k_pool_rows(hidden, pool_row, out, B, d, (hipStream_t)stream);
}
extern "C" int gget_op_scatter_rows_f32(const float* src, const int32_t* pool_row, void* dhidden, int B, int d, void* stream) {
  GGET_REQUIRE(src && pool_row && dhidden && B > 0 && d > 0, "scatter_rows_f32: null argument or empty shape");
  return k_scatter_rows_f32(src, pool_row, dhidden, B, d, (hipStream_t)stream);
}
extern "C" int gget_op_head_linear_fwd(const void* x, void* a, const void* w, const void* bias, void* y, float* y32, int B, int Din,
                                       int Dout, int layer, void* stream) {
  GGET_REQUIRE(x && a && w && y && B > 0 && Din > 0 && Dout > 0, "head_linear_fwd: null argument or empty shape");
  return k_head_linear_fwd(x, a, w, bias, y, y32, B, Din, Dout, layer, gget_engine::elem_drop(0.f, 0), (hipStream_t)stream);
}
extern "C" int gget_op_head_linear_bwd(const float* dy, const void* x, const void* a, const void* w, float* dw, float* dbias, float* dx,
                                       int B, int Din, int Dout, int layer, void* stream) {
  GGET_REQUIRE(dy && x && a && w && dw && dx && B > 0 && Din > 0 && Dout > 0, "head_linear_bwd: null argument or empty shape");
  return k_head_linear_bwd(dy, x, a, w, dw, dbias, dx, B, Din, Dout, layer, gget_engine::elem_drop(0.f, 0), (hipStream_t)stream);
}
extern "C" int gget_op_lengths(const int64_t* mask, const int64_t* ids, int ldF, int pad_id, int32_t* key_len, int32_t* pool_row, int B,
                               int S, void* stream) {
  GGET_REQUIRE((key_len || pool_row) && (!pool_row || ids) && B > 0 && S > 0 && (!ids || ldF >= 1), "lengths: null argument or empty shape");
  return k_lengths(mask, ids, ldF, pad_id, key_len, pool_row, B, S, (hipStream_t)stream);
}
extern "C" int gget_op_sum_lengths(const int32_t* key_len, int B, int32_t* out, void* stream) {
  GGET_REQUIRE(key_len && out && B > 0, "sum_lengths: null argument or empty shape");
  return k_sum_lengths(key_len, B, out, (hipStream_t)stream, nullptr);
}
extern "C" int gget_op_varlen_plan(const int64_t* ids, int ldF, int F, const int64_t* pos, int32_t* key_len, int32_t* pool_row, int32_t* cu,
                                   int64_t* ids_c, int64_t* pos_c, int32_t* row_b, int32_t* pad2c, int32_t* c2p, int32_t* status, int B,
                                   int S, int tc, int t_rows, int pad_id, int32_t* long_list, void* stream) {
  GGET_REQUIRE(ids && key_len && cu && ids_c && pos_c && row_b && pad2c && c2p && status, "varlen_plan: null argument");
  GGET_REQUIRE(B > 0 && S > 0 && F >= 1 && ldF >= F && tc >= 0 && t_rows >= tc, "varlen_plan: bad shape B %d S %d F %d ldF %d tc %d t_rows %d", B, S,
               F, ldF, tc, t_rows);
  return k_varlen_plan(ids, ldF, F, pos, key_len, pool_row, cu, ids_c, pos_c, row_b, pad2c, c2p, status, B, S, tc, t_rows, pad_id,
                       (hipStream_t)stream, long_list);
}
extern "C" int gget_op_rows_to_grid(const void* src, const int32_t* pad2c, void* out, int64_t n_pos, int d, void* stream) {
  GGET_REQUIRE(src && pad2c && out && n_pos >= 0 && d > 0 && d % 8 == 0, "rows_to_grid: null argument or bad shape (d must be a multiple of 8)");
  return k_rows_to_grid(src, pad2c, out, (long)n_pos, d, (hipStream_t)stream);
}
extern "C" uint64_t gget_op_head_compact_ws_bytes(int T) { return T > 0 ? (uint64_t)k_head_compact_ws_bytes(T) : 0; }
extern "C" int gget_op_head_compact(const int64_t* labels, int T, int n, int32_t* cnt, int32_t* m_off, int32_t* l_off, int32_t* counts,
                                    int32_t* row_idx, int32_t* sel_src, int32_t* sel_label, int32_t* sel_tok, int32_t* ws,
                                    int32_t* slot_hist, void* stream) {
  GGET_REQUIRE(cnt && m_off && l_off && counts && row_idx && sel_src && sel_label && sel_tok && ws, "head_compact: null argument");
  GGET_REQUIRE(T > 0 && n >= 1, "head_compact: bad shape T %d n %d", T, n);
  return k_head_compact(labels, T, n, cnt, m_off, l_off, counts, row_idx, sel_src, sel_label, sel_tok, ws, slot_hist, (hipStream_t)stream);
}
extern "C" int gget_op_head_slot_sort(const int32_t* sel_src, const int32_t* row_idx, const int32_t* lm_count, int32_t* slot_state,
                                      int32_t* a_tok, int32_t* a_cell, int32_t* c_l, int32_t* cellpos, int32_t* tile_off, int32_t* total_p,
                                      int cap, int n, int64_t slot_elems, int tile_rows, void* stream) {
  GGET_REQUIRE(sel_src && row_idx && lm_count && slot_state && a_tok && a_cell && c_l && cellpos && tile_off && total_p,
               "head_slot_sort: null argument");
  GGET_REQUIRE(cap > 0 && n >= 1 && tile_rows > 0 && slot_elems >= 0, "head_slot_sort: bad shape cap %d n %d tile_rows %d", cap, n, tile_rows);
  return k_head_slot_sort(sel_src, row_idx, lm_count, slot_state, a_tok, a_cell, c_l, cellpos, tile_off, total_p, cap, n, (long)slot_elems,
                          tile_rows, (hipStream_t)stream);
}
extern "C" int gget_op_head_cell_sum(const void* dxs, const int32_t* cellpos, const int32_t* cnt, const int32_t* l_off, const int32_t* pad2c,
                                     void* dhid, int TP, int d, int pad_row, void* stream) {
  GGET_REQUIRE(dxs && cellpos && cnt && l_off && dhid && TP > 0 && d > 0 && d % 8 == 0 && pad_row >= 0,
               "head_cell_sum: null argument or bad shape (d must be a multiple of 8)");
  return k_head_cell_sum(dxs, cellpos, cnt, l_off, pad2c, dhid, TP, d, pad_row, (hipStream_t)stream);
}
extern "C" int gget_op_gather_rows(const void* src, const int32_t* idx, const int32_t* count, void* dst, int cap, int d, int scatter,
                                   void* stream) {
  GGET_REQUIRE(src && idx && count && dst && cap >= 0 && d > 0 && d % 8 == 0, "gather_rows: null argument or bad shape (d must be a multiple of 8)");
  return k_gather_rows(src, idx, count, dst, cap, d, scatter, (hipStream_t)stream);
}
extern "C" int gget_op_gather_rows_remap(const void* src, int32_t* idx, const int32_t* count, const int32_t* pad2c, void* dst, int cap, int d,
                                         int pad_row, int32_t* status, void* stream) {
  GGET_REQUIRE(src && idx && count && pad2c && dst && cap >= 0 && d > 0 && d % 8 == 0 && pad_row >= 0,
               "gather_rows_remap: null argument or bad shape (d must be a multiple of 8)");
  return k_gather_rows_remap(src, idx, count, pad2c, dst, cap, d, pad_row, status, (hipStream_t)stream);
}
extern "C" int gget_op_sample_mask_wgt(const int64_t* labels, float* w, int B, int cells, void* stream) {
  GGET_REQUIRE(labels && w && B >= 0 && cells >= 1, "sample_mask_wgt: null argument or empty shape");
  return k_sample_mask_wgt(labels, w, B, cells, (hipStream_t)stream);
}
extern "C" int gget_op_raw_blend(const float* raw, const int64_t* labels, int n, int first_only, const void* tok, void* out, int32_t* flag,
                                 int T, int e, const int32_t* rows_map, int n_logical, void* stream) {
  GGET_REQUIRE(raw && tok && out && flag && T >= 0 && e > 0 && (!labels || n >= 1) && (!rows_map || n_logical >= 0),
               "raw_blend: null argument or bad shape");
  return k_raw_blend(raw, labels, n, first_only != 0, tok, out, flag, T, e, (hipStream_t)stream, rows_map, n_logical);
}
extern "C" int gget_op_raw_tok_grad(const void* dx, const int32_t* flag, float* dtok, int T, int e, void* stream) {
  GGET_REQUIRE(dx && flag && dtok && T >= 0 && e > 0, "raw_tok_grad: null argument or empty shape");
  return k_raw_tok_grad(dx, flag, dtok, T, e, (hipStream_t)stream);
}
extern "C" int gget_op_gemm_indexed(int mode, const void* A, const void* B, void* C, int M_cap, int N, int K, int lda, int ldb, int ldc,
                                    const int32_t* m_dev, const int32_t* a_rows, const int32_t* b_tile_off, int b_tile_rows,
                                    const int32_t* c_rows, void* stream) {
  GGET_REQUIRE(A && B && C && M_cap >= 0 && N > 0 && K > 0, "gemm_indexed: null argument or empty shape");
  if (!a_rows && !b_tile_off)
    return gget_gemm_single(mode, GGET_EPI_NONE, A, B, C, nullptr, M_cap, N, K, lda, ldb, ldc, m_dev, nullptr, 1, (hipStream_t)stream, false,
                            c_rows);
  GGET_REQUIRE(b_tile_rows == 128 || b_tile_rows == 256, "gemm_indexed: b_tile_rows %d is neither 128 nor 256", b_tile_rows);
  GemmGroup g;
  memset(&g, 0, sizeof(g));
  g.count = 1;
  GemmProblem& p = g.p[0];
  p.A = static_cast<const bf16_t*>(A); p.B = static_cast<const bf16_t*>(B); p.C = C;
  p.M = M_cap; p.N = N; p.K = K; p.lda = lda; p.ldb = ldb; p.ldc = ldc;
  p.m_dev = m_dev;
  p.a_rows = a_rows; p.b_tile_off = b_tile_off; p.c_rows = c_rows;
  p.b_tile_rows = b_tile_rows;
  return gget_gemm_launch(mode, GGET_EPI_NONE, g, 1, (hipStream_t)stream);
}


namespace {

struct RcclApi {
  ncclResult_t (*GetUniqueId)(ncclUniqueId*) = nullptr;
  ncclResult_t (*CommInitRank)(ncclComm_t*, int, ncclUniqueId, int) = nullptr;
  ncclResult_t (*CommDestroy)(ncclComm_t) = nullptr;
  ncclResult_t (*AllReduce)(const void*, void*, size_t, ncclDataType_t, ncclRedOp_t, ncclComm_t, hipStream_t) = nullptr;
  ncclResult_t (*ReduceScatter)(const void*, void*, size_t, ncclDataType_t, ncclRedOp_t, ncclComm_t, hipStream_t) = nullptr;
  ncclResult_t (*AllGather)(const void*, void*, size_t, ncclDataType_t, ncclComm_t, hipStream_t) = nullptr;
  ncclResult_t (*GroupStart)() = nullptr;
  ncclResult_t (*GroupEnd)() = nullptr;
  const char* (*GetErrorString)(ncclResult_t) = nullptr;
  bool ok = false;
  char why[256] = "symbols missing";
};

RcclApi* rccl() {
  static RcclApi api;
  static bool tried = false;
  if (!tried) {
    tried = true;
    void* lib = dlopen("librccl.so.1", RTLD_NOW | RTLD_GLOBAL);
    if (!lib) lib = dlopen("librccl.so", RTLD_NOW | RTLD_GLOBAL);
    if (!lib) {
      const char* e = dlerror();
      snprintf(api.why, sizeof(api.why), "%s", e ? e : "dlopen failed");
    }
    if (lib) {
      api.GetUniqueId = reinterpret_cast<decltype(api.GetUniqueId)>(dlsym(lib, "ncclGetUniqueId"));
      api.CommInitRank = reinterpret_cast<decltype(api.CommInitRank)>(dlsym(lib, "ncclCommInitRank"));
      api.CommDestroy = reinterpret_cast<decltype(api.CommDestroy)>(dlsym(lib, "ncclCommDestroy"));
// ... 228 lines not shown
```

graph-gpt_amd/csrc/kernels.h:

```cpp
#pragma once
#include <hip/hip_runtime.h>
#include "../../include/gget.h"
#include "common.h"

constexpr int kAccumCopies = 8;
constexpr uint64_t kAccumCopyMax = 8192;
struct GgetSegment {
  uint64_t src;
  uint64_t dst;
  uint64_t count;
  uint64_t copies;
  uint64_t stride;
};

int k_embed_fwd(const int64_t* ids, const void* emb, const void* gate, void* out, int T, int F, int ldF, int d,
                hipStream_t st, ElemDropArg E = ElemDropArg{0, 1.f, 0});
int k_elem_dropout(void* x, long T, int n, unsigned stream, ElemDropArg E, hipStream_t st);
#define GGET_DROP_STREAM_RAW 60u
int k_raw_blend(const float* raw, const int64_t* labels, int n, bool first_only, const void* tok, void* out, int32_t* flag, int T, int e,
                hipStream_t st, const int32_t* rows_map = nullptr, int n_logical = 0);
int k_raw_tok_grad(const void* dx, const int32_t* flag, float* dtok, int T, int e, hipStream_t st);
int k_embed_long_ratio(const int64_t* ids, void* x, int T, int F, int ldF, int d, hipStream_t st);
int k_sample_mask_wgt(const int64_t* labels, float* w, int B, int cells, hipStream_t st);
int k_embed_bwd(const int64_t* ids, const void* dx, const void* emb, const void* gate, float* demb, float* dgate, int T,
                int F, int ldF, int d, int V, int pad_id, int32_t* sort_ws, hipStream_t st, ElemDropArg E = ElemDropArg{0, 1.f, 0});
inline size_t k_embed_bwd_ws_elems(size_t ncell, size_t V) { return 3 * V + 1 + 2 * ncell; }
int k_embed_count(const int64_t* ids, void* cnt, int T, int F, int ldF, int ldc, int pad_id, hipStream_t st);
inline bool k_embed_dense_ok(int V, bool gated) { return !gated && ((V + 63) / 64) * 64 <= 1024; }
constexpr int kEmbDenseSplit = 8;
int k_rmsnorm_fwd(const void* x, const void* w, void* y, float* rstd, int T, int d, float eps, hipStream_t st);
int k_det_scratch(size_t floats, float** out);
int k_ordered_colsum(float* part, int nblk, int d, float* dst, hipStream_t st);
int k_rmsnorm_bwd(const void* dy, const void* x, const void* w, const float* rstd, const void* dres, void* dx,
                  float* dw_accum, int T, int d, hipStream_t st, int copies = 1, uint64_t copy_stride = 0);
int k_rmsnorm_dw(const void* dy, const void* x, const float* rstd, float* dw_accum, int T, int d, hipStream_t st, int copies = 1,
                 uint64_t copy_stride = 0);
int k_rope(void* qkv, const float* cos_tab, const float* sin_tab, const int64_t* position_ids, int T, int S, int H,
           int inverse, hipStream_t st);
int k_rope_table(float* cos_tab, float* sin_tab, int max_pos, float theta, hipStream_t st);
int k_rope_range_table(const int64_t* pos, float* cos_t, float* sin_t, int64_t* ids, int B, int S, float range, float theta,
                       hipStream_t st);
int k_geglu_fwd(const void* gu, void* h, int T, int ff, hipStream_t st);
int k_geglu_bwd(const void* gu, const void* dh, void* dgu, int T, int ff, hipStream_t st);
int k_lengths(const int64_t* mask, const int64_t* ids, int ldF, int pad_id, int32_t* key_len, int32_t* pool_row, int B,
              int S, hipStream_t st);
int k_varlen_plan(const int64_t* ids, int ldF, int F, const int64_t* pos, int32_t* key_len, int32_t* pool_row, int32_t* cu,
                  int64_t* ids_c, int64_t* pos_c, int32_t* row_b, int32_t* pad2c, int32_t* c2p, int32_t* status, int B, int S, int tc,
                  int t_rows, int pad_id, hipStream_t st, int32_t* long_list = nullptr);
int k_clamp_positions(const int64_t* pos, int64_t* out, int32_t* flag, long n, int max_pos, hipStream_t st);
int k_head_slot_sort(const int32_t* sel_src, const int32_t* row_idx, const int32_t* lm_count, int32_t* slot_state, int32_t* a_tok,
                     int32_t* a_cell, int32_t* c_l, int32_t* cellpos, int32_t* tile_off, int32_t* total_p, int cap, int n, long slot_elems,
                     int tile_rows, hipStream_t st);
int k_head_cell_sum(const void* dxs, const int32_t* cellpos, const int32_t* cnt, const int32_t* l_off, const int32_t* pad2c, void* dhid,
                    int TP, int d, int pad_row, hipStream_t st);
int k_poison_loss(const int32_t* flag, float* loss, hipStream_t st);
int k_sum_lengths(const int32_t* key_len, int B, int32_t* out, hipStream_t st, int32_t* host_out = nullptr);
int k_head_compact(const int64_t* labels, int T, int n, int32_t* cnt, int32_t* m_off, int32_t* l_off, int32_t* counts,
                   int32_t* row_idx, int32_t* sel_src, int32_t* sel_label, int32_t* sel_tok, int32_t* blk_tot, int32_t* slot_hist,
                   hipStream_t st);
size_t k_head_compact_ws_bytes(int T);
int k_gather_rows(const void* src, const int32_t* idx, const int32_t* count, void* dst, int cap, int d, int scatter,
                  hipStream_t st);
int k_gather_rows_remap(const void* src, int32_t* idx, const int32_t* count, const int32_t* pad2c, void* dst, int cap, int d, int pad_row,
                        int32_t* status, hipStream_t st);
int k_ce_fwd_bwd(const void* logits, int ld, const int32_t* labels, const int32_t* sel_tok, const float* sample_wgt, int S,
                 const int32_t* n_rows_dev, int n_rows_cap, int V, float* loss_sum, void* dlogits, float scale_base,
                 int mean_over_rows, float* loss_out, hipStream_t st, float focal_gamma = 0.f, float* loss_part = nullptr,
                 int loss_part_cap = 0);
int k_score_fwd(const void* hidden, const int32_t* pool_row, const void* w, const void* bias, float* logits,
                void* pooled_h, int B, int C, int d, hipStream_t st);
int k_tok_score_fwd(const void* hidden, const void* w, const void* bias, float* logits, int T, int C, int d, hipStream_t st);
int k_tok_ce(const float* logits, const int64_t* labels, float* dl, float* stat, float* loss_out, int T, int C, hipStream_t st,
             const int32_t* rows_map = nullptr, int n_logical = 0);
int k_copy_from_host(const void* src_host_mapped, void* dst, size_t bytes, hipStream_t st);
int k_rows_to_grid(const void* src, const int32_t* pad2c, void* out, long n_pos, int d, hipStream_t st);
int k_scatter_rows_map_f32(const float* src, const int32_t* rows_map, float* dst, int T, int C, int n_logical, hipStream_t st);
int k_tok_score_bwd(const float* dl, const float* stat, const void* hidden, const void* w, float* dw, float* dbias, void* dhidden, int T,
                    int C, int d, hipStream_t st);
int k_tok_intra_fwd(const void* hidden, const int32_t* row_start, const int64_t* cls_idx, float* logits, int B, int C, int d,
                    hipStream_t st);
int k_tok_intra_bwd(const float* dl, const float* stat, const void* hidden, const int32_t* row_start, const int64_t* cls_idx,
                    void* dhidden, int B, int C, int d, hipStream_t st);
int k_intra_plan(const int64_t* cls_idx, const int32_t* key_len, const int32_t* cu, int32_t* row_start, int64_t* cls_safe, int32_t* flag,
                 int B, int S, int C, hipStream_t st);
int k_pool_rows(const void* hidden, const int32_t* pool_row, void* out, int B, int d, hipStream_t st);
int k_head_linear_fwd(const void* x, void* a, const void* w, const void* bias, void* y, float* y32, int B, int Din, int Dout,
                      int layer, ElemDropArg E, hipStream_t st);
int k_head_linear_bwd(const float* dy, const void* x, const void* a, const void* w, float* dw, float* dbias, float* dx, int B,
                      int Din, int Dout, int layer, ElemDropArg E, hipStream_t st);
int k_scatter_rows_f32(const float* src, const int32_t* pool_row, void* dhidden, int B, int d, hipStream_t st);
int k_auc_loss(const float* logits, const int64_t* labels, int B, int C, int num_neg, unsigned seed, float* loss_out,
               float* dlogits, int32_t* lists, hipStream_t st);
int k_task_loss(const float* logits, const void* labels, const float* sample_wgt, int problem, int B, int C,
                float* loss_out, float* dlogits, hipStream_t st);
int k_score_bwd(const float* dlogits, const void* hidden, const int32_t* pool_row, const void* w, float* dw, float* dbias,
                void* dhidden, int B, int C, int d, hipStream_t st);
int k_grad_sqnorm(const void* g, size_t n, float* ws, hipStream_t st, bool grad_f32 = false);
inline size_t k_grad_sqnorm_ws_bytes() { return (16 + 1024) * sizeof(float); }
struct GgetSqChunk { uint64_t off; uint64_t cnt; };
int k_grad_sqnorm_chunks(const void* g, const GgetSqChunk* chunks_dev, int nchunks, const float* extra, int nextra, float* ws, hipStream_t st,
                         bool grad_f32 = false);
int k_grad_sqnorm_partials(const void* g, const GgetSqChunk* chunks_dev, const int32_t* slot_dev, int nchunks, float* out, hipStream_t st,
                           bool grad_f32 = false);
int k_grad_sqnorm_slots(const float* slots, const int32_t* slot_of_dev, int n, float* ws, hipStream_t st);
struct GgetAdamwArgs {
  float *master, *m, *v;
  const void* grad;
  bool grad_f32;
  void* param;
  float lr, beta1, beta2, eps, wd;
  int step;
  float max_norm, grad_scale;
  const float* sqnorm;
  float* gnorm_out;
  bool skip_nonfinite;
  float* ema;
  float ema_decay;
};
int k_adamw(const GgetAdamwArgs& a, size_t n, hipStream_t st);
constexpr int kAdamwItemElems = 2048;
int k_adamw_items(const GgetAdamwArgs& a, const GgetSqChunk* items_dev, int nitems, hipStream_t st);
int k_grad_accumulate(const void* grad, float* acc, size_t n, bool first, hipStream_t st);
int k_ema_lerp(const float* master, float* ema, size_t n, float d, hipStream_t st);
int k_ema_lerp_items(const float* master, float* ema, const GgetSqChunk* items_dev, int nitems, float d, hipStream_t st);
constexpr int kZeroRanges = 6;
struct GgetZeroRanges {
  void* ptr[kZeroRanges];
  size_t bytes[kZeroRanges];
  int n;
  void add(void* p, size_t b) { if (b && n < kZeroRanges) { ptr[n] = p; bytes[n] = b; ++n; } }
};
int k_zero_ranges(const GgetZeroRanges& R, hipStream_t st);
int k_f32_to_bf16(const float* src, void* dst, size_t n, hipStream_t st);
int k_slab_reduce(const float* slabs, long slab_stride, int nslab, void* dst, size_t n, hipStream_t st, bool f32_out = false);
int k_convert_segments(const float* scratch, void* grads, const GgetSegment* segs_dev, int nseg, hipStream_t st);

int k_attn_fwd(const void* qkv, const int32_t* key_len, void* out, float* lse, int B, int S, int H, int causal,
               const float* cos_tab, const float* sin_tab, const int64_t* position_ids, float dropout_p,
               unsigned dropout_seed, hipStream_t st, const int32_t* key_lo = nullptr, const int32_t* key_hi = nullptr,
               const int32_t* row_base = nullptr, const int32_t* long_list = nullptr);
int k_attn_probs(const void* qkv, const float* lse, const int32_t* key_len, const int32_t* row_base, const int32_t* key_lo,
                 const int32_t* key_hi, void* out, int B, int S, int H, int causal, float dropout_p, unsigned dropout_seed, hipStream_t st);
int k_qkv_grid(const void* src, const int32_t* key_len, const int32_t* row_base, const int32_t* key_lo, const int32_t* key_hi, void* out,
// ... 29 lines not shown
```

graph-gpt_amd/csrc/kernels.hip:

```cpp
#include "common.h"
#include "kernels.h"

static float* g_det_scratch = nullptr;
static size_t g_det_bytes = 0;

namespace {

constexpr int kBlock = 256;

__device__ __forceinline__ uint4 ldg16(const bf16_t* p) { return *reinterpret_cast<const uint4*>(p); }
__device__ __forceinline__ void stg16(bf16_t* p, const uint4& v) {
  typedef unsigned u4nt __attribute__((ext_vector_type(4)));
  __builtin_nontemporal_store(u4nt{v.x, v.y, v.z, v.w}, reinterpret_cast<u4nt*>(p));
}

__global__ void __launch_bounds__(128) embed_fwd_kernel(const int64_t* __restrict__ ids, const bf16_t* __restrict__ emb,
                                                        const bf16_t* __restrict__ gate, bf16_t* __restrict__ out,
                                                        int T, int F, int ldF, int d, ElemDropArg E) {
  const int t = blockIdx.x;
  const int64_t* row = ids + (size_t)t * ldF;
  for (int c = threadIdx.x; c * 8 < d; c += blockDim.x) {
    float acc[8] = {0, 0, 0, 0, 0, 0, 0, 0};
    for (int f0 = 0; f0 < F; f0 += 4) {
      uint4 r[4], gr[4];
// ... 2540 lines not shown
  else
    hipLaunchKernelGGL(rmsnorm_dw_kernel<4>, dim3(grid), dim3(kBlock), 4 * d * sizeof(float), st, (const bf16_t*)dy, (const bf16_t*)x, rstd,
                       dw_accum, T, d, copies, copy_stride, part);
  GGET_LAUNCH_CHECK();
  if (part) return k_ordered_colsum(part, grid, d, dw_accum, st);
  return 0;
}

int k_det_scratch(size_t floats, float** out) {
  if (g_det_bytes < floats * sizeof(float)) {
    if (g_det_scratch) GGET_HIP_CHECK(hipFree(g_det_scratch));
    g_det_scratch = nullptr;
    g_det_bytes = 0;
    GGET_HIP_CHECK(hipMalloc(&g_det_scratch, floats * sizeof(float)));
    g_det_bytes = floats * sizeof(float);
  }
  *out = g_det_scratch;
  return 0;
}

int k_ordered_colsum(float* part, int nblk, int d, float* dst, hipStream_t st) {
  constexpr int kPer = 64;
  const int nseg = (nblk + kPer - 1) / kPer;
  float* seg = part + (size_t)nblk * d;
  hipLaunchKernelGGL(ordered_colsum_kernel, dim3((d + 63) / 64, nseg), dim3(kBlock), 0, st, part, nblk, d, kPer, seg, 0);
  hipLaunchKernelGGL(ordered_colsum_kernel, dim3((d + 63) / 64, 1), dim3(kBlock), 0, st, seg, nseg, d, nseg, dst, 1);
  GGET_LAUNCH_CHECK();
  return 0;
}

int k_rope(void* qkv, const float* cos_tab, const float* sin_tab, const int64_t* position_ids, int T, int S, int H,
           int inverse, hipStream_t st) {
  GGET_REQUIRE(qkv && cos_tab && sin_tab, "rope: null argument");
  GGET_REQUIRE(T >= 0 && H >= 1 && S >= 1, "rope: bad shape T %d S %d H %d", T, S, H);
  if (T == 0) return 0;
  hipLaunchKernelGGL(rope_kernel, dim3(grid_for((long)T * 8 * H)), dim3(kBlock), 0, st, (bf16_t*)qkv, cos_tab, sin_tab,
                     position_ids, T, S, H, inverse);
  GGET_LAUNCH_CHECK();
  return 0;
}

int k_rope_table(float* cos_tab, float* sin_tab, int max_pos, float theta, hipStream_t st) {
  hipLaunchKernelGGL(rope_table_kernel, dim3((max_pos * 32 + 255) / 256), dim3(256), 0, st, cos_tab, sin_tab, max_pos,
                     theta);
  GGET_LAUNCH_CHECK();
  return 0;
}

int k_rope_range_table(const int64_t* pos, float* cos_t, float* sin_t, int64_t* ids, int B, int S, float range, float theta,
                       hipStream_t st) {
  if (B * S == 0) return 0;
  hipLaunchKernelGGL(rope_range_table_kernel, dim3(B), dim3(kBlock), 0, st, pos, cos_t, sin_t, ids, S, range, theta);
  GGET_LAUNCH_CHECK();
  return 0;
}

int k_geglu_fwd(const void* gu, void* h, int T, int ff, hipStream_t st) {
  GGET_REQUIRE(gu && h, "geglu_fwd: null argument");
  GGET_REQUIRE(T >= 0 && ff > 0 && ff % 8 == 0, "geglu_fwd: bad shape T %d ff %d (ff must be a multiple of 8)", T, ff);
  if (T == 0) return 0;
  hipLaunchKernelGGL(geglu_fwd_kernel, dim3(grid_for((long)T * (ff / 8))), dim3(kBlock), 0, st, (const bf16_t*)gu,
                     (bf16_t*)h, (long)T, ff);
  GGET_LAUNCH_CHECK();
  return 0;
}

int k_geglu_bwd(const void* gu, const void* dh, void* dgu, int T, int ff, hipStream_t st) {
  GGET_REQUIRE(gu && dh && dgu, "geglu_bwd: null argument");
  GGET_REQUIRE(T >= 0 && ff > 0 && ff % 8 == 0, "geglu_bwd: bad shape T %d ff %d (ff must be a multiple of 8)", T, ff);
  if (T == 0) return 0;
  hipLaunchKernelGGL(geglu_bwd_kernel, dim3(grid_for((long)T * (ff / 8))), dim3(kBlock), 0, st, (const bf16_t*)gu,
                     (const bf16_t*)dh, (bf16_t*)dgu, (long)T, ff);
  GGET_LAUNCH_CHECK();
  return 0;
}

int k_lengths(const int64_t* mask, const int64_t* ids, int ldF, int pad_id, int32_t* key_len, int32_t* pool_row, int B,
              int S, hipStream_t st) {
  hipLaunchKernelGGL(lengths_kernel, dim3(B), dim3(64), 0, st, mask, ids, ldF, pad_id, key_len, pool_row, B, S);
  GGET_LAUNCH_CHECK();
  return 0;
}

__global__ void __launch_bounds__(1024) varlen_scan_kernel(int32_t* __restrict__ key_len, int32_t* __restrict__ cu,
                                                           int32_t* __restrict__ pool_row, int32_t* __restrict__ status, int B, int S,
                                                           int expect_total, int32_t* __restrict__ long_list) {
  __shared__ int wsum[16];
  __shared__ int lsum[16];
  __shared__ int carry_s, lcarry_s;
  const int tid = threadIdx.x, lane = tid & 63, wave = tid >> 6;
  if (tid == 0) { carry_s = 0; lcarry_s = 0; }
  __syncthreads();
  for (int b0 = 0; b0 < B; b0 += 1024) {
    const int b = b0 + tid;
    const int v = b < B ? key_len[b] : 0;
    int x = v;
#pragma unroll
    for (int o = 1; o < 64; o <<= 1) {
      const int y = __shfl_up(x, o, 64);
      if (lane >= o) x += y;
    }
    if (lane == 63) wsum[wave] = x;
    __syncthreads();
    int base = carry_s;
    for (int w = 0; w < wave; ++w) base += wsum[w];
    int len = 0;
    if (b < B) {
      const int start = min(base + x - v, expect_total);
      len = min(v, expect_total - start);
      cu[b] = start;
      if (len != v) key_len[b] = len;
      if (pool_row) {
        const int pidx = pool_row[b] - b * S;
        pool_row[b] = min(start + max(min(pidx, len - 1), 0), max(expect_total - 1, 0));
      }
    }
    const bool is_long = len > 32 && len <= 64;
    const unsigned long long bal = __ballot(is_long);
    if (lane == 0) lsum[wave] = __popcll(bal);
    __syncthreads();
    if (long_list && is_long) {
      int lpos = lcarry_s;
      for (int w = 0; w < wave; ++w) lpos += lsum[w];
      lpos += __popcll(bal & ((1ull << lane) - 1ull));
      long_list[1 + lpos] = b;
      long_list[1 + B + lpos] = cu[b];
      long_list[1 + 2 * B + lpos] = len;
    }
    __syncthreads();
    if (tid == 1023) {
      carry_s = base + x;
      int lt = lcarry_s;
      for (int w = 0; w < 16; ++w) lt += lsum[w];
      lcarry_s = lt;
    }
    __syncthreads();
  }
  if (tid == 0) {
    if (long_list) long_list[0] = lcarry_s;
    cu[B] = min(carry_s, expect_total);
    status[0] = carry_s == expect_total ? 0 : 1;
    if (carry_s != expect_total) status[2] = 1;
  }
}
__global__ void __launch_bounds__(kBlock) varlen_fill_kernel(const int64_t* __restrict__ ids, int ldF, int F, const int64_t* __restrict__ pos,
                                                             const int32_t* __restrict__ key_len, const int32_t* __restrict__ cu,
                                                             int64_t* __restrict__ ids_c, int64_t* __restrict__ pos_c,
                                                             int32_t* __restrict__ row_b, int32_t* __restrict__ pad2c,
                                                             int32_t* __restrict__ c2p, int B, int S, int tc, int t_rows, int64_t pad_id) {
  const long i = (long)blockIdx.x * kBlock + threadIdx.x;
  const long TP = (long)B * S;
  if (i < TP) {
    const int b = (int)(i / S), sq = (int)(i % S);
    if (sq < key_len[b]) {
      const int r = cu[b] + sq;
      for (int f = 0; f < F; ++f) ids_c[(size_t)r * F + f] = ids[(size_t)i * ldF + f];
      pos_c[r] = pos ? pos[i] : (int64_t)sq;
      row_b[r] = b;
      pad2c[i] = r;
      c2p[r] = (int)i;
    } else {
      pad2c[i] = -1;
    }
  } else if (i < TP + (t_rows - tc)) {
    const int r = tc + (int)(i - TP);
    for (int f = 0; f < F; ++f) ids_c[(size_t)r * F + f] = pad_id;
    pos_c[r] = 0;
    row_b[r] = 0;
    c2p[r] = (int)i;
  }
}
__global__ void __launch_bounds__(1024) sum_lengths_kernel(const int32_t* __restrict__ key_len, int B, int32_t* __restrict__ out,
                                                           int32_t* __restrict__ host_out) {
  __shared__ int tot;
  if (threadIdx.x == 0) tot = 0;
  __syncthreads();
  int v = 0;
  for (int b = threadIdx.x; b < B; b += 1024) v += key_len[b];
  if (v) atomicAdd(&tot, v);
  __syncthreads();
  if (threadIdx.x == 0) {
    *out = tot;
    if (host_out) __hip_atomic_store(host_out, tot, __ATOMIC_RELEASE, __HIP_MEMORY_SCOPE_SYSTEM);
  }
}

__global__ void __launch_bounds__(kBlock) clamp_positions_kernel(const int64_t* __restrict__ pos, int64_t* __restrict__ out,
                                                                 int32_t* __restrict__ flag, long n, int max_pos) {
  bool bad = false;
  for (long i = (long)blockIdx.x * kBlock + threadIdx.x; i < n; i += (long)gridDim.x * kBlock) {
    const int64_t v = pos[i];
    bad |= v < 0 || v >= max_pos;
    out[i] = v < 0 ? 0 : (v >= max_pos ? max_pos - 1 : v);
  }
  if (__any(bad) && (threadIdx.x & 63) == 0) *flag = 1;
}
int k_clamp_positions(const int64_t* pos, int64_t* out, int32_t* flag, long n, int max_pos, hipStream_t st) {
  if (n == 0) return 0;
  hipLaunchKernelGGL(clamp_positions_kernel, dim3(grid_for(n, kBlock, 1024)), dim3(kBlock), 0, st, pos, out, flag, n, max_pos);
  GGET_LAUNCH_CHECK();
  return 0;
}

int k_varlen_plan(const int64_t* ids, int ldF, int F, const int64_t* pos, int32_t* key_len, int32_t* pool_row, int32_t* cu,
                  int64_t* ids_c, int64_t* pos_c, int32_t* row_b, int32_t* pad2c, int32_t* c2p, int32_t* status, int B, int S, int tc,
                  int t_rows, int pad_id, hipStream_t st, int32_t* long_list) {
  hipLaunchKernelGGL(varlen_scan_kernel, dim3(1), dim3(1024), 0, st, key_len, cu, pool_row, status, B, S, tc, long_list);
  const long n = (long)B * S + (t_rows - tc);
  hipLaunchKernelGGL(varlen_fill_kernel, dim3((unsigned)((n + kBlock - 1) / kBlock)), dim3(kBlock), 0, st, ids, ldF, F, pos, key_len, cu,
                     ids_c, pos_c, row_b, pad2c, c2p, B, S, tc, t_rows, (int64_t)pad_id);
  GGET_LAUNCH_CHECK();
  return 0;
}
__global__ void __launch_bounds__(kBlock) copy_from_host_kernel(const unsigned char* __restrict__ src, unsigned char* __restrict__ dst, size_t n) {
  const size_t n16 = n / 16;
  for (size_t i = (size_t)blockIdx.x * kBlock + threadIdx.x; i < n16; i += (size_t)gridDim.x * kBlock)
    reinterpret_cast<uint4*>(dst)[i] = reinterpret_cast<const uint4*>(src)[i];
  if (blockIdx.x == 0)
    for (size_t i = n16 * 16 + threadIdx.x; i < n; i += kBlock) dst[i] = src[i];
}
int k_copy_from_host(const void* src_host_mapped, void* dst, size_t bytes, hipStream_t st) {
  if (bytes == 0) return 0;
  GGET_REQUIRE((((uintptr_t)src_host_mapped | (uintptr_t)dst) & 15) == 0, "copy_from_host: 16-byte aligned buffers");
  hipLaunchKernelGGL(copy_from_host_kernel, dim3(grid_for((long)(bytes / 16 + 1), kBlock, 256)), dim3(kBlock), 0, st, (const unsigned char*)src_host_mapped,
                     (unsigned char*)dst, bytes);
  GGET_LAUNCH_CHECK();
  return 0;
}

__global__ void __launch_bounds__(kBlock) rows_to_grid_kernel(const bf16_t* __restrict__ src, const int32_t* __restrict__ pad2c,
                                                              bf16_t* __restrict__ out, long n_pos, int d) {
  const int cpr = d / 8;
  for (long i = (long)blockIdx.x * kBlock + threadIdx.x; i < n_pos * cpr; i += (long)gridDim.x * kBlock) {
    const long pos = i / cpr;
    const int c = (int)(i % cpr);
    const int r = pad2c[pos];
    uint4 v = make_uint4(0u, 0u, 0u, 0u);
    if (r >= 0) v = *reinterpret_cast<const uint4*>(src + (size_t)r * d + c * 8);
    *reinterpret_cast<uint4*>(out + (size_t)pos * d + c * 8) = v;
  }
}
int k_rows_to_grid(const void* src, const int32_t* pad2c, void* out, long n_pos, int d, hipStream_t st) {
  if (n_pos == 0) return 0;
  hipLaunchKernelGGL(rows_to_grid_kernel, dim3(grid_for(n_pos * (d / 8), kBlock, 4096)), dim3(kBlock), 0, st, (const bf16_t*)src, pad2c, (bf16_t*)out,
                     n_pos, d);
  GGET_LAUNCH_CHECK();
  return 0;
}

__global__ void poison_loss_kernel(const int32_t* __restrict__ flag, float* __restrict__ loss) {
  if (*flag) *loss = __builtin_nanf("");
}
int k_poison_loss(const int32_t* flag, float* loss, hipStream_t st) {
  hipLaunchKernelGGL(poison_loss_kernel, dim3(1), dim3(1), 0, st, flag, loss);
  GGET_LAUNCH_CHECK();
  return 0;
}
int k_sum_lengths(const int32_t* key_len, int B, int32_t* out, hipStream_t st, int32_t* host_out) {
  hipLaunchKernelGGL(sum_lengths_kernel, dim3(1), dim3(1024), 0, st, key_len, B, out, host_out);
  GGET_LAUNCH_CHECK();
  return 0;
}

int k_head_slot_sort(const int32_t* sel_src, const int32_t* row_idx, const int32_t* lm_count, int32_t* slot_state, int32_t* a_tok,
                     int32_t* a_cell, int32_t* c_l, int32_t* cellpos, int32_t* tile_off, int32_t* total_p, int cap, int n, long slot_elems,
                     int tile_rows, hipStream_t st) {
  if (n > 32) { gget_set_error("slot-sorted head: next_n_token %d > 32", n); return 2; }
  hipLaunchKernelGGL(slot_fill_kernel, dim3((cap + kBlock * kFillItems - 1) / (kBlock * kFillItems)), dim3(kBlock), 0, st, sel_src, row_idx, lm_count, slot_state, a_tok,
                     a_cell, c_l, cellpos, tile_off, total_p, cap, n, slot_elems, tile_rows);
  GGET_LAUNCH_CHECK();
  return 0;
}
int k_head_cell_sum(const void* dxs, const int32_t* cellpos, const int32_t* cnt, const int32_t* l_off, const int32_t* pad2c, void* dhid,
                    int TP, int d, int pad_row, hipStream_t st) {
  hipLaunchKernelGGL(head_cell_sum_kernel, dim3((TP + kBlock / 64 - 1) / (kBlock / 64)), dim3(kBlock), 0, st, (const bf16_t*)dxs, cellpos, cnt,
                     l_off, pad2c, (bf16_t*)dhid, TP, d, pad_row);
  GGET_LAUNCH_CHECK();
  return 0;
}

int k_head_compact(const int64_t* labels, int T, int n, int32_t* cnt, int32_t* m_off, int32_t* l_off, int32_t* counts,
                   int32_t* row_idx, int32_t* sel_src, int32_t* sel_label, int32_t* sel_tok, int32_t* blk_tot, int32_t* slot_hist,
                   hipStream_t st) {
  const int g = (T + kBlock - 1) / kBlock;
  hipLaunchKernelGGL(head_count_kernel, dim3(g), dim3(kBlock), 0, st, labels, cnt, blk_tot, T, n);
  hipLaunchKernelGGL(head_fill_kernel, dim3(g), dim3(kBlock), 0, st, labels, cnt, blk_tot, m_off, l_off, counts, row_idx, sel_src,
                     sel_label, sel_tok, n <= 32 ? slot_hist : nullptr, T, n);
  GGET_LAUNCH_CHECK();
  return 0;
}
size_t k_head_compact_ws_bytes(int T) { return (size_t)((T + kBlock - 1) / kBlock) * 8; }

int k_gather_rows(const void* src, const int32_t* idx, const int32_t* count, void* dst, int cap, int d, int scatter,
                  hipStream_t st) {
  if (cap == 0) return 0;
  hipLaunchKernelGGL(gather_rows_kernel, dim3(grid_for((long)cap * (d / 8))), dim3(kBlock), 0, st, (const bf16_t*)src,
                     idx, count, (bf16_t*)dst, cap, d, scatter);
  GGET_LAUNCH_CHECK();
  return 0;
}

int k_gather_rows_remap(const void* src, int32_t* idx, const int32_t* count, const int32_t* pad2c, void* dst, int cap, int d, int pad_row,
                        int32_t* status, hipStream_t st) {
  if (cap == 0) return 0;
  hipLaunchKernelGGL(gather_rows_remap_kernel, dim3(grid_for((long)cap * 64)), dim3(kBlock), 0, st, (const bf16_t*)src, idx, count, pad2c,
                     (bf16_t*)dst, cap, d, pad_row, status);
  GGET_LAUNCH_CHECK();
  return 0;
}

int k_ce_fwd_bwd(const void* logits, int ld, const int32_t* labels, const int32_t* sel_tok, const float* sample_wgt, int S,
                 const int32_t* n_rows_dev, int n_rows_cap, int V, float* loss_sum, void* dlogits, float scale_base,
                 int mean_over_rows, float* loss_out, hipStream_t st, float focal_gamma, float* loss_part, int loss_part_cap) {
  const bool vec = (ld % 8) == 0 && ((uintptr_t)logits & 15) == 0 && ((uintptr_t)dlogits & 15) == 0 && !menu().ce_generic;
  const dim3 grid(grid_for(n_rows_cap, 4 * 8, 2048));
  const bool parts = menu().ce_parts && loss_part && n_rows_cap > 0 && vec && ld <= 2048 && (int)grid.x <= loss_part_cap;
  if (!parts) GGET_HIP_CHECK(hipMemsetAsync(loss_sum, 0, sizeof(float), st));
  if (n_rows_cap > 0) {
    float* lp = parts ? loss_part : nullptr;
#define GGET_CE_ARGS (const bf16_t*)logits, ld, labels, sel_tok, sample_wgt, S, n_rows_dev, n_rows_cap, V, loss_sum, \
                     (bf16_t*)dlogits, scale_base, mean_over_rows, focal_gamma
    if (vec && ld <= 512) hipLaunchKernelGGL(ce_rows_kernel<1>, grid, dim3(kBlock), 0, st, GGET_CE_ARGS, lp);
    else if (vec && ld <= 1024) hipLaunchKernelGGL(ce_rows_kernel<2>, grid, dim3(kBlock), 0, st, GGET_CE_ARGS, lp);
    else if (vec && ld <= 2048) hipLaunchKernelGGL(ce_rows_kernel<4>, grid, dim3(kBlock), 0, st, GGET_CE_ARGS, lp);
    else hipLaunchKernelGGL(ce_fwd_bwd_kernel, grid, dim3(kBlock), 0, st, GGET_CE_ARGS);
#undef GGET_CE_ARGS
  }
  if (loss_out || parts)
    hipLaunchKernelGGL(finalize_loss_kernel, dim3(1), dim3(256), 0, st, loss_sum, n_rows_dev, n_rows_cap, scale_base, mean_over_rows,
                       loss_out, parts ? loss_part : nullptr, (int)grid.x);
  GGET_LAUNCH_CHECK();
  return 0;
}

int k_tok_score_fwd(const void* hidden, const void* w, const void* bias, float* logits, int T, int C, int d, hipStream_t st) {
  GGET_REQUIRE(d % 64 == 0 && d <= 64 * kTokMaxCols, "token-level head: d=%d unsupported", d);
  if (T == 0) return 0;
  const int rows_per_block = (kBlock / 64) * kTokRows;
  hipLaunchKernelGGL(tok_score_fwd_kernel, dim3((T + rows_per_block - 1) / rows_per_block), dim3(kBlock), 0, st, (const bf16_t*)hidden,
                     (const bf16_t*)w, (const bf16_t*)bias, logits, T, C, d);
  GGET_LAUNCH_CHECK();
  return 0;
}
__global__ void __launch_bounds__(kBlock) scatter_rows_map_f32_kernel(const float* __restrict__ src, const int32_t* __restrict__ rows_map,
                                                                      float* __restrict__ dst, long T, int C, int n_logical) {
  for (long w = (long)blockIdx.x * kBlock + threadIdx.x; w < T * C; w += (long)gridDim.x * kBlock) {
    const long t = w / C;
    const int lt = rows_map[t];
    if (lt < n_logical) dst[(size_t)lt * C + (w % C)] = src[w];
  }
}
int k_scatter_rows_map_f32(const float* src, const int32_t* rows_map, float* dst, int T, int C, int n_logical, hipStream_t st) {
  if (T == 0) return 0;
  hipLaunchKernelGGL(scatter_rows_map_f32_kernel, dim3(grid_for((long)T * C, kBlock, 2048)), dim3(kBlock), 0, st, src, rows_map, dst, (long)T, C,
                     n_logical);
  GGET_LAUNCH_CHECK();
  return 0;
}
int k_tok_ce(const float* logits, const int64_t* labels, float* dl, float* stat, float* loss_out, int T, int C, hipStream_t st,
             const int32_t* rows_map, int n_logical) {
  GGET_HIP_CHECK(hipMemsetAsync(stat, 0, 4 * sizeof(float), st));
  if (T > 0)
    hipLaunchKernelGGL(tok_ce_kernel, dim3(grid_for(T, kBlock, 1024)), dim3(kBlock), 0, st, logits, labels, dl, stat, T, C, rows_map,
                       rows_map ? n_logical : T);
  hipLaunchKernelGGL(tok_ce_final_kernel, dim3(1), dim3(1), 0, st, stat, loss_out);
  GGET_LAUNCH_CHECK();
  return 0;
}
int k_tok_score_bwd(const float* dl, const float* stat, const void* hidden, const void* w, float* dw, float* dbias, void* dhidden, int T,
                    int C, int d, hipStream_t st) {
  if (T == 0) return 0;
  const int rows_per_block = (kBlock / 64) * kTokRows;
  hipLaunchKernelGGL(tok_score_bwd_dx_kernel, dim3((T + rows_per_block - 1) / rows_per_block), dim3(kBlock), 0, st, dl, stat,
                     (const bf16_t*)w, (bf16_t*)dhidden, T, C, d);
// ... 358 lines not shown
```

graph-gpt_amd/csrc/menu.h:

```cpp
#pragma once

struct LaunchMenu {
  int gemm_variant;
  int gemm_lds_headroom;
  int gemm_split_last;
  int gemm_stagger_ticks;
  int gemm_ablate;
  int gemm_cu_reserve;
  int gemm_num_cu;
  int gemm_no_persist;
  int gemm_no_dyn;
  int gemm_no_256;
  int gemm_bk64;
  int gemm_192;
  int gemm_super;
  int attn_by_sample;
  int attn_big;
  int attn_dense;
  int attn_small;
  int attn_fused;
  int attn_fused_min_s;
  int attn_stg128;
  int attn_oproj;
  int attn_oproj_off;
  int head_sorted;
  int head_dense;
  int head_tile;
  int no_head_scatter_fusion;
  int no_geglu_fusion;
  int no_ls_norm_fusion;
  int ls_norm_bwd_wide;
  int no_varlen;
  int count_copy;
  int embed_sorted;
  int occupy_fat;
  int deterministic;
  int rms_wide;
  int rms_rows;
  int ce_parts;
  int ce_generic;
  int link_grid;
};

enum : int {
  kGemmNoKsplitNd = 1,
  kGemmNoKsplitWgrad = 2,
  kGemmNo192Rows = 4,
  kGemmNoSplitLast = 8,
  kGemmKsplit128Only = 16,
  kGemmOneBlockPerCu = 32,
  kGemmKsplitDma8 = 128,
  kGemmAreaRule = 512,
};

struct MenuRow {
  int LaunchMenu::*field;
  int key;
  const char* env;
  bool env_presence;
  int def;
  const char* meaning;
};

inline constexpr MenuRow kMenuRows[] = {
    {&LaunchMenu::gemm_variant, 1, "GGET_GEMM_VARIANT", false, 0, "bit mask of GEMM kernel variants (kGemm*)"},
    {&LaunchMenu::gemm_lds_headroom, 2, "GGET_GEMM_LDS_HEADROOM", false, 1, "LDS headroom of the 128x192 / 192x128 tiles: 0 4-slot rings, 1 3-slot, 2 also one block per CU"},
    {&LaunchMenu::gemm_split_last, 3, "GGET_GEMM_SPLIT_LAST", false, 0, "1: split the K range of the last, partial round's tiles among the idle blocks"},
    {&LaunchMenu::deterministic, 4, "GGET_DETERMINISTIC", false, 0, "1: reproducible mode, RMSNorm weight gradients summed in block order"},
    {&LaunchMenu::gemm_stagger_ticks, 5, "GGET_GEMM_STAGGER", false, 0, "MODE 2 GEMM launches: start delay of a CU's second workgroup (100 MHz ticks)"},
    {&LaunchMenu::gemm_ablate, 7, "GGET_GEMM_ABLATE", false, 0, "GEMM diagnostics: 1 no LDS-DMA, 2 no MFMA, 4 no C store, 32 no epilogue (timing only)"},
    {&LaunchMenu::head_dense, 8, nullptr, false, 0, "1: SMTP head as a dense projection through all slots"},
    {&LaunchMenu::head_tile, 9, nullptr, false, 0, "SMTP head slot tile rows: 0 automatic, 128 / 256 forced"},
    {&LaunchMenu::attn_oproj_off, 10, nullptr, false, 0, "1: S <= 32 attention, o projection, RMSNorm as three launches"},
    {&LaunchMenu::ls_norm_bwd_wide, 11, "GGET_LS_NORM_BWD_WIDE", false, 0, "1: fused RMSNorm + LayerScale backward in its 16-byte-chunk form for every width"},
    {&LaunchMenu::rms_wide, 13, "GGET_RMS_WIDE", false, 1, "0: short RMSNorm backward launches in 4-wave blocks instead of one 16-wave block per CU"},
    {&LaunchMenu::ce_parts, 14, "GGET_CE_PARTS", false, 1, "0: cross-entropy adds its loss with one atomic per block instead of per-block partial sums"},
    {&LaunchMenu::gemm_cu_reserve, 15, nullptr, false, 0, "CUs every GEMM plan leaves free for a collective's workgroups"},
    {&LaunchMenu::occupy_fat, 16, nullptr, false, 0, "1: gget_debug_occupy's stand-in takes RCCL's register footprint"},
    {&LaunchMenu::link_grid, 18, nullptr, false, 0, "> 0: most workgroups a streaming launch of the link metrics takes (0: 1024)"},
    {&LaunchMenu::gemm_num_cu, 0, "GGET_GEMM_NUM_CU", false, 0, "> 0: GEMM plans pretend the chip has this many CUs"},
    {&LaunchMenu::gemm_no_persist, 0, "GGET_GEMM_NO_PERSIST", true, 0, "set: no persistent GEMM kernels"},
    {&LaunchMenu::gemm_no_dyn, 0, "GGET_GEMM_NO_DYN", true, 0, "set: no persistent GEMM kernels for device-sized launches"},
    {&LaunchMenu::gemm_no_256, 0, "GGET_GEMM_NO_256", true, 0, "set: no 256x256 GEMM tiles"},
    {&LaunchMenu::gemm_bk64, 0, "GGET_GEMM_BK64", false, 1, "0: 256x256 NT tiles with 32-deep instead of 64-deep K-tiles"},
    {&LaunchMenu::gemm_192, 0, "GGET_GEMM_192", false, 1, "0: no 128x192 / 192x192 GEMM tiles"},
    {&LaunchMenu::gemm_super, 0, "GGET_GEMM_SUPER", false, 0, "> 0: tile-order supergroup size of every GEMM launch"},
    {&LaunchMenu::attn_by_sample, 0, "GGET_ATTN_BY_SAMPLE", false, 1, "0: var-len 32 < S <= 64 attention keyed by S instead of every sample's own rows"},
    {&LaunchMenu::attn_big, 0, "GGET_ATTN_BIG", false, 1, "0: S >= 256 attention on the register-prefetch kernels"},
    {&LaunchMenu::attn_dense, 0, "GGET_ATTN_DENSE", false, 1, "0: no dense attention forward for S >= 512"},
    {&LaunchMenu::attn_small, 0, "GGET_ATTN_SMALL", false, 1, "0: no per-sample attention backward for S <= 64"},
    {&LaunchMenu::attn_fused, 0, "GGET_ATTN_FUSED", false, 1, "0: long-sequence attention backward as two kernels instead of one pass"},
    {&LaunchMenu::attn_fused_min_s, 0, "GGET_ATTN_FUSED_MIN_S", false, 256, "sequence length from which the one-pass attention backward runs"},
    {&LaunchMenu::attn_stg128, 0, "GGET_ATTN_STG128", false, 1, "0: S >= 512 dK / dV kernel with 64-row instead of 128-row stages"},
    {&LaunchMenu::attn_oproj, 0, "GGET_ATTN_OPROJ", false, 1, "0: S <= 32 attention, o projection, RMSNorm as three launches"},
    {&LaunchMenu::head_sorted, 0, "GGET_HEAD_SORTED", false, 1, "0: SMTP head as a dense projection through all slots"},
    {&LaunchMenu::no_head_scatter_fusion, 0, "GGET_NO_HEAD_SCATTER_FUSION", true, 0, "set: SMTP head rows scattered by their own launch (implies the dense head)"},
    {&LaunchMenu::no_geglu_fusion, 0, "GGET_NO_GEGLU_FUSION", true, 0, "set: GEGLU as GEMM + element-wise kernel"},
    {&LaunchMenu::no_ls_norm_fusion, 0, "GGET_NO_LS_NORM_FUSION", true, 0, "set: LayerScale residual and the next RMSNorm as separate launches"},
    {&LaunchMenu::no_varlen, 0, "GGET_NO_VARLEN", true, 0, "set: the padded token grid instead of the var-len layout"},
    {&LaunchMenu::count_copy, 0, "GGET_COUNT_COPY", false, 0, "1: token count back by device-to-host copy + event instead of a polled host word"},
    {&LaunchMenu::embed_sorted, 20, "GGET_EMBED_SORTED", true, 0, "set: embedding backward always as the sorted scatter-add"},
    {&LaunchMenu::rms_rows, 0, "GGET_RMS_ROWS", false, 4, "RMSNorm backward rows per wave"},
    {&LaunchMenu::ce_generic, 19, "GGET_CE_GENERIC", true, 0, "set: cross-entropy never on the vectorised row kernels"},
};

extern LaunchMenu g_menu;
extern thread_local const LaunchMenu* t_call_menu;
inline const LaunchMenu& menu() { return t_call_menu ? *t_call_menu : g_menu; }
```

include/gget.h:

```cpp
#ifndef GGET_H_
#define GGET_H_

#include <stddef.h>
#include <stdint.h>

#ifdef __cplusplus
extern "C" {
#endif

#define GGET_KIND_PRETRAIN 0
#define GGET_KIND_TASK 1

#define GGET_PROBLEM_SINGLE_LABEL 0
#define GGET_PROBLEM_REGRESSION_L1 1
#define GGET_PROBLEM_REGRESSION_MSE 2
#define GGET_PROBLEM_TOKEN_CE 5
#define GGET_PROBLEM_TOKEN_CE_INTRA 6
#define GGET_PROBLEM_AUC 4
#define GGET_PROBLEM_MULTI_LABEL 3

typedef struct gget_config_t {
  int32_t kind;
  int32_t vocab_size;
  int32_t hidden_size;
// ... 234 lines not shown
int gget_op_attn_oproj_bwd(const void* dxn, const void* x_mid, const void* norm_w, const float* rstd, const void* dres, void* dx_mid,
                           float* dw_accum, int copies, uint64_t copy_stride, const void* wot_packed, const void* qkv, const float* lse,
                           const int32_t* key_len, const int32_t* row_base, void* dqkv, int B, int S, int H, int causal, const float* cos_tab,
                           const float* sin_tab, const int64_t* position_ids, float dropout_p, uint32_t dropout_seed, int t_rows,
                           void* stream, int32_t* taken, void* dattn_long);
int gget_op_attn_fwd_ranges(const void* qkv, const int32_t* key_lo, const int32_t* key_hi, void* out, float* lse, int B, int S,
                            int H, int causal, float dropout_p, uint32_t dropout_seed, void* stream);
int gget_op_attn_bwd_ranges(const void* qkv, const void* out, const void* dout, const float* lse, const int32_t* key_lo,
                            const int32_t* key_hi, void* dqkv, float* delta_ws, int B, int S, int H, int causal,
                            float dropout_p, uint32_t dropout_seed, void* stream);
int gget_op_ranges_from_mask3d(const int64_t* mask3d, int32_t* key_lo, int32_t* key_hi, int B, int S, void* stream);
int gget_op_attn_probs(const void* qkv, const float* lse, const int32_t* key_len, const int32_t* row_base, const int32_t* key_lo,
                       const int32_t* key_hi, void* out, int B, int S, int H, int causal, float dropout_p, uint32_t dropout_seed,
                       void* stream);
int gget_op_attn_bwd_fused(const void* qkv, const void* out, const void* dout, const float* lse, const int32_t* key_len,
                           const int32_t* key_lo, const int32_t* key_hi, void* dqkv, float* delta_ws, void* dq_ws, int B, int S,
                           int H, int causal, float dropout_p, uint32_t dropout_seed, void* stream);
int gget_op_gateup_geglu(const void* x, const void* wgu, void* gu, void* h, int T, int d, int ff, void* stream);
int gget_op_down_dgrad_geglu(const void* dy, const void* wdown, const void* gu, void* dgu, void* dh_scratch, int T, int d, int ff,
                             void* stream);
int gget_op_geglu_fwd(const void* gu, void* h, int T, int ff, void* stream);
int gget_op_geglu_bwd(const void* gu, const void* dh, void* dgu, int T, int ff, void* stream);
int gget_op_ce_fwd_bwd(const void* logits, int ld, const int32_t* labels, const float* row_wgt, const int32_t* n_rows_dev,
                       int n_rows_cap, int V, float* loss_sum, void* dlogits, float grad_scale_base, int mean_over_rows,
                       void* stream);

int gget_op_rmsnorm_bwd_copies(const void* dy, const void* x, const void* w, const float* rstd, const void* dres, void* dx, float* dw_accum,
                               int T, int d, int copies, uint64_t copy_stride, void* stream);
int gget_op_rmsnorm_dw(const void* dy, const void* x, const float* rstd, float* dw_accum, int T, int d, int copies, uint64_t copy_stride,
                       void* stream);
int gget_op_ls_rmsnorm_fwd(const void* res, const void* y, const void* lam, void* out, const void* w, void* xn, float* rstd, int T, int d,
                           float eps, void* stream);
int gget_op_accum_layout(int d, int* copies, uint64_t* copy_stride);
int gget_op_rmsnorm_bwd_ls(const void* dy, const void* x, const void* w, const float* rstd, const void* dres, void* dx, float* dw_accum,
                           const void* y, const void* lam, void* dsc, float* dlam_accum, int T, int d, void* stream);
int gget_op_ce_full(const void* logits, int ld, const int32_t* labels, const int32_t* sel_tok, const float* sample_wgt, int S,
                    const int32_t* n_rows_dev, int n_rows_cap, int V, float* loss_sum, void* dlogits, float scale_base, int mean_over_rows,
                    float* loss_out, float focal_gamma, float* loss_part, int loss_part_cap, void* stream);

int gget_op_rope_table(float* cos_tab, float* sin_tab, int max_pos, float theta, void* stream);
int gget_op_rope_range_table(const int64_t* pos, float* cos_tab, float* sin_tab, int64_t* ids, int B, int S, float range, float theta,
                             void* stream);
int gget_op_clamp_positions(const int64_t* pos, int64_t* out, int32_t* flag, int64_t n, int max_pos, void* stream);
int gget_op_embed_long_ratio(const int64_t* ids, void* x, int T, int F, int ldF, int d, void* stream);

int gget_op_score_fwd(const void* hidden, const int32_t* pool_row, const void* w, const void* bias, float* logits, void* pooled_h,
                      int B, int C, int d, void* stream);
int gget_op_score_bwd(const float* dlogits, const void* hidden, const int32_t* pool_row, const void* w, float* dw, float* dbias,
                      void* dhidden, int B, int C, int d, void* stream);
int gget_op_tok_score_fwd(const void* hidden, const void* w, const void* bias, float* logits, int T, int C, int d, void* stream);
int gget_op_tok_ce(const float* logits, const int64_t* labels, float* dl, float* stat, float* loss_out, int T, int C,
                   const int32_t* rows_map, int n_logical, void* stream);
int gget_op_tok_score_bwd(const float* dl, const float* stat, const void* hidden, const void* w, float* dw, float* dbias, void* dhidden,
                          int T, int C, int d, void* stream);
int gget_op_tok_intra_fwd(const void* hidden, const int32_t* row_start, const int64_t* cls_idx, float* logits, int B, int C, int d,
                          void* stream);
int gget_op_tok_intra_bwd(const float* dl, const float* stat, const void* hidden, const int32_t* row_start, const int64_t* cls_idx,
                          void* dhidden, int B, int C, int d, void* stream);
int gget_op_task_loss(const float* logits, const void* labels, const float* sample_wgt, int problem, int B, int C, float* loss_out,
                      float* dlogits, void* stream);
int gget_op_auc_loss(const float* logits, const int64_t* labels, int B, int C, int num_neg, uint32_t seed, float* loss_out,
                     float* dlogits, int32_t* lists, void* stream);
int gget_op_pool_rows(const void* hidden, const int32_t* pool_row, void* out, int B, int d, void* stream);
int gget_op_scatter_rows_f32(const float* src, const int32_t* pool_row, void* dhidden, int B, int d, void* stream);
int gget_op_head_linear_fwd(const void* x, void* a, const void* w, const void* bias, void* y, float* y32, int B, int Din, int Dout,
                            int layer, void* stream);
int gget_op_head_linear_bwd(const float* dy, const void* x, const void* a, const void* w, float* dw, float* dbias, float* dx, int B,
                            int Din, int Dout, int layer, void* stream);

int gget_op_lengths(const int64_t* mask, const int64_t* ids, int ldF, int pad_id, int32_t* key_len, int32_t* pool_row, int B, int S,
                    void* stream);
int gget_op_sum_lengths(const int32_t* key_len, int B, int32_t* out, void* stream);
int gget_op_varlen_plan(const int64_t* ids, int ldF, int F, const int64_t* pos, int32_t* key_len, int32_t* pool_row, int32_t* cu,
                        int64_t* ids_c, int64_t* pos_c, int32_t* row_b, int32_t* pad2c, int32_t* c2p, int32_t* status, int B, int S, int tc,
                        int t_rows, int pad_id, int32_t* long_list, void* stream);
int gget_op_rows_to_grid(const void* src, const int32_t* pad2c, void* out, int64_t n_pos, int d, void* stream);
uint64_t gget_op_head_compact_ws_bytes(int T);
int gget_op_head_compact(const int64_t* labels, int T, int n, int32_t* cnt, int32_t* m_off, int32_t* l_off, int32_t* counts,
                         int32_t* row_idx, int32_t* sel_src, int32_t* sel_label, int32_t* sel_tok, int32_t* ws, int32_t* slot_hist,
                         void* stream);
int gget_op_head_slot_sort(const int32_t* sel_src, const int32_t* row_idx, const int32_t* lm_count, int32_t* slot_state, int32_t* a_tok,
                           int32_t* a_cell, int32_t* c_l, int32_t* cellpos, int32_t* tile_off, int32_t* total_p, int cap, int n,
                           int64_t slot_elems, int tile_rows, void* stream);
int gget_op_head_cell_sum(const void* dxs, const int32_t* cellpos, const int32_t* cnt, const int32_t* l_off, const int32_t* pad2c,
                          void* dhid, int TP, int d, int pad_row, void* stream);
int gget_op_gather_rows(const void* src, const int32_t* idx, const int32_t* count, void* dst, int cap, int d, int scatter, void* stream);
int gget_op_gather_rows_remap(const void* src, int32_t* idx, const int32_t* count, const int32_t* pad2c, void* dst, int cap, int d,
                              int pad_row, int32_t* status, void* stream);
int gget_op_sample_mask_wgt(const int64_t* labels, float* w, int B, int cells, void* stream);
int gget_op_raw_blend(const float* raw, const int64_t* labels, int n, int first_only, const void* tok, void* out, int32_t* flag, int T,
                      int e, const int32_t* rows_map, int n_logical, void* stream);
int gget_op_raw_tok_grad(const void* dx, const int32_t* flag, float* dtok, int T, int e, void* stream);
int gget_op_gemm_indexed(int mode, const void* A, const void* B, void* C, int M_cap, int N, int K, int lda, int ldb, int ldc,
                         const int32_t* m_dev, const int32_t* a_rows, const int32_t* b_tile_off, int b_tile_rows, const int32_t* c_rows,
                         void* stream);

size_t gget_op_rank_metrics_workspace(int n, int C);
int gget_op_rank_metrics(const float* scores, int ld_s, const float* labels, int ld_y, int n, int C, int64_t* n_pos, int64_t* n_neg,
                         uint64_t* auc2, double* ap_sum, int32_t* n_bad, void* workspace, size_t workspace_bytes, void* stream);

size_t gget_op_link_hits_workspace(int n);
int gget_op_link_hits(const float* scores, const int64_t* labels, int n, int64_t K, int64_t* n_pos, int64_t* n_neg, float* kth, int64_t* hits,
                      int32_t* n_bad, void* workspace, size_t workspace_bytes, void* stream);
size_t gget_op_link_mrr_workspace(int n);
int gget_op_link_mrr(const float* scores, const int64_t* labels, const int64_t* idx, int n, int cnt_neg, int groups, int64_t* n_pos,
                     int64_t* n_neg, int32_t* optimistic, int32_t* pessimistic, int64_t* hits_1_3_10, double* mrr_sum, int32_t* n_bad,
                     void* workspace, size_t workspace_bytes, void* stream);

#define GGET_CLUSTER_MAX_C 2048
int gget_op_cluster_metrics(const void* pred_or_logits, int is_logits, const int64_t* labels, const int64_t* raw_node_idx, int B, int S,
                            int C, int64_t* y_pred, int32_t* counts, int64_t* totals, void* stream);

#ifdef __cplusplus
}
#endif
#endif
```

Before: 819,700 graph-tokens/s.

## Fuse per-step index planning into one persistent step-plan kernel

```diff
diff --git a/graph-gpt_amd/_lib.py b/graph-gpt_amd/_lib.py
--- a/graph-gpt_amd/_lib.py
+++ b/graph-gpt_amd/_lib.py
@@ -170,6 +170,8 @@
     "gget_op_head_compact_ws_bytes": (u64, [i32]),
     "gget_op_head_compact": (i32, [vp, i32, i32, vp, vp, vp, vp, vp, vp, vp, vp, vp, vp, vp]),
     "gget_op_head_slot_sort": (i32, [vp, vp, vp, vp, vp, vp, vp, vp, vp, vp, i32, i32, i64, i32, vp]),
+    "gget_op_step_plan_ws_bytes": (u64, [i32]),
+    "gget_op_step_plan": (i32, [vp, vp, vp, vp, i32, i32, i32, i32, i32, i32, i32] + [vp] * 24 + [i64, i32, vp, vp]),
     "gget_op_head_cell_sum": (i32, [vp, vp, vp, vp, vp, vp, i32, i32, i32, vp]),
     "gget_op_gather_rows": (i32, [vp, vp, vp, vp, i32, i32, i32, vp]),
     "gget_op_gather_rows_remap": (i32, [vp, vp, vp, vp, vp, i32, i32, i32, vp, vp]),
@@ -198,8 +200,8 @@
 KEY_GEMM_VARIANT, KEY_GEMM_LDS_HEADROOM, KEY_GEMM_SPLIT_LAST, KEY_DETERMINISTIC, KEY_GEMM_STAGGER = 1, 2, 3, 4, 5
 KEY_GEMM_ABLATE, KEY_HEAD_DENSE, KEY_HEAD_TILE, KEY_ATTN_OPROJ_OFF, KEY_LS_NORM_BWD_WIDE = 7, 8, 9, 10, 11
 KEY_RMS_WIDE, KEY_CE_PARTS, KEY_GEMM_CU_RESERVE, KEY_OCCUPY_FAT, KEY_LINK_GRID, KEY_CE_GENERIC = 13, 14, 15, 16, 18, 19
-KEY_EMBED_SORTED = 20
-MENU_KEYS = (1, 2, 3, 4, 5, 7, 8, 9, 10, 11, 13, 14, 15, 16, 18, 19, 20)
+KEY_EMBED_SORTED, KEY_STEP_PLAN = 20, 21
+MENU_KEYS = (1, 2, 3, 4, 5, 7, 8, 9, 10, 11, 13, 14, 15, 16, 18, 19, 20, 21)
 GEMM_NO_KSPLIT_ND, GEMM_NO_KSPLIT_WGRAD, GEMM_NO_192_ROWS, GEMM_NO_SPLIT_LAST, GEMM_KSPLIT_128_ONLY, GEMM_ONE_BLOCK_PER_CU = 1, 2, 4, 8, 16, 32
 GEMM_KSPLIT_DMA8, GEMM_AREA_RULE = 128, 512
 
diff --git a/graph-gpt_amd/csrc/engine.hip b/graph-gpt_amd/csrc/engine.hip
--- a/graph-gpt_amd/csrc/engine.hip
+++ b/graph-gpt_amd/csrc/engine.hip
@@ -183,6 +183,7 @@
   uint64_t vl_long;
   uint64_t wo_pack = 0, wot_pack = 0;
   uint64_t pos_safe;
+  uint64_t sp_ws = 0;
   uint64_t sk_ws;
   uint64_t head_x[6] = {0}, head_a[5] = {0}, head_d[2] = {0};
   uint64_t total;
@@ -273,6 +274,7 @@
     const uint64_t n = c.next_n_token, Vp = align_up(c.vocab_size, 64);
     w.cnt = b.take(T * 4);
     w.hc_tot = b.take(k_head_compact_ws_bytes((int)T));
+    w.sp_ws = b.take(k_step_plan_ws_bytes((int)T));
     w.m_off = b.take(T * 4);
     w.l_off = b.take(T * 4);
     w.row_idx = b.take(T * 4);
@@ -474,6 +476,9 @@
   }
   std::function<int(hipStream_t)> presync_work;
   bool presync_done = false;
+  std::function<int(hipStream_t, int, int32_t*, const int64_t*)> plan_work;
+  bool plan_done = false;
+  bool step_plan_off = false;
   hipEvent_t count_event = nullptr;
   unsigned auc_seed = 0;
   bool fwd_valid = false;
@@ -776,9 +781,18 @@
   int32_t cls_clamped = 0;
   GGET_HIP_CHECK(hipMemcpyAsync(&cls_clamped, st + 4, 4, hipMemcpyDeviceToHost, (hipStream_t)stream));
   GGET_HIP_CHECK(hipMemsetAsync(st + 1, 0, 8, (hipStream_t)stream));
-  GGET_HIP_CHECK(hipMemsetAsync(st + 4, 0, 4, (hipStream_t)stream));
+  int32_t plan_gave_up = 0;
+  GGET_HIP_CHECK(hipMemcpyAsync(&plan_gave_up, st + 5, 4, hipMemcpyDeviceToHost, (hipStream_t)stream));
+  GGET_HIP_CHECK(hipMemsetAsync(st + 4, 0, 8, (hipStream_t)stream));
   GGET_HIP_CHECK(hipStreamSynchronize((hipStream_t)stream));
   if (cls_clamped) out[0] |= 2;
+  if (plan_gave_up) {
+    h->step_plan_off = true;
+    if (h->ws.sp_ws) GGET_HIP_CHECK(hipMemset(h->wsp<int32_t>(h->ws.sp_ws), 0, 16));
+    gget_set_error("a step plan launch gave up waiting for its scan block: the results since the last status read are invalid; "
+                   "the separate index launches run from now on");
+    return 2;
+  }
   return 0;
 }
 
@@ -1380,13 +1394,33 @@
     if (early_done) return 0;
     early_done = true;
     if (int e = pack_o_weights()) return e;
-    if (h->presync_work) {
+    if (h->presync_work && !h->plan_done) {
       if (int e = h->presync_work(st)) return e;
       h->presync_done = true;
     }
     return 0;
   };
-  if (mask_is_3d) {
+  auto need_host_word = [&]() -> int {
+    if (h->host_word) return 0;
+    GGET_HIP_CHECK(hipHostMalloc(reinterpret_cast<void**>(&h->host_word), 64, hipHostMallocMapped | hipHostMallocCoherent));
+    GGET_HIP_CHECK(hipHostGetDevicePointer(reinterpret_cast<void**>(&h->host_word_dev), h->host_word, 0));
+    return 0;
+  };
+  constexpr int32_t kNoCount = INT32_MIN;
+  const bool want_varlen = allow_varlen && varlen_enabled() && (tc_hint > 0 || tc_hint == GGET_TOKENS_AUTO) && !mask_is_3d && mask != nullptr;
+  const bool use_plan = want_varlen && h->plan_work && menu().step_plan && !h->step_plan_off && !(h->rope_range > 0.f) &&
+                        tc_hint < (1L << 31) && !(tc_hint == GGET_TOKENS_AUTO && menu().count_copy);
+  h->plan_done = false;
+  if (use_plan) {
+    const bool count_here = tc_hint == GGET_TOKENS_AUTO;
+    if (count_here) {
+      if (int e = need_host_word()) return e;
+      __atomic_store_n(h->host_word, kNoCount, __ATOMIC_RELEASE);
+    }
+    if (int e = h->plan_work(st, count_here ? -1 : (int)tc_hint, count_here ? h->host_word_dev : nullptr, pos)) return e;
+    h->plan_done = true;
+    h->presync_done = true;
+  } else if (mask_is_3d) {
     GGET_REQUIRE(mask != nullptr && c.kind == GGET_KIND_PRETRAIN, "a 3-D (packed) attention mask needs the pre-train model and a mask");
     if (int e = k_ranges_from_mask3d(mask, h->wsp<int32_t>(h->ws.key_lo), h->wsp<int32_t>(h->ws.key_hi), B, S, st)) return e;
   } else if (int e = k_lengths(mask, c.kind == GGET_KIND_TASK ? ids : nullptr, ldF, c.pad_token_id,
@@ -1394,18 +1428,15 @@
                                c.kind == GGET_KIND_TASK ? h->wsp<int32_t>(h->ws.pool_row) : nullptr, B, S, st)) {
     return e;
   }
-  if (allow_varlen && varlen_enabled() && (tc_hint > 0 || tc_hint == GGET_TOKENS_AUTO) && !mask_is_3d && mask != nullptr) {
+  if (want_varlen) {
     long tc = tc_hint;
     if (tc_hint == GGET_TOKENS_AUTO) {
       int32_t* dst = h->wsp<int32_t>(h->ws.vl_status) + 3;
-      if (!h->host_word) {
-        GGET_HIP_CHECK(hipHostMalloc(reinterpret_cast<void**>(&h->host_word), 64, hipHostMallocMapped | hipHostMallocCoherent));
-        GGET_HIP_CHECK(hipHostGetDevicePointer(reinterpret_cast<void**>(&h->host_word_dev), h->host_word, 0));
-      }
-      const bool count_copy = menu().count_copy != 0;
-      constexpr int32_t kNoCount = INT32_MIN;
-      if (!count_copy) __atomic_store_n(h->host_word, kNoCount, __ATOMIC_RELEASE);
-      if (int e = k_sum_lengths(h->wsp<int32_t>(h->ws.key_len), B, dst, st, count_copy ? nullptr : h->host_word_dev)) return e;
+      if (int e = need_host_word()) return e;
+      const bool count_copy = menu().count_copy != 0 && !h->plan_done;
+      if (!count_copy && !h->plan_done) __atomic_store_n(h->host_word, kNoCount, __ATOMIC_RELEASE);
+      if (!h->plan_done)
+        if (int e = k_sum_lengths(h->wsp<int32_t>(h->ws.key_len), B, dst, st, count_copy ? nullptr : h->host_word_dev)) return e;
       if (count_copy) {
         GGET_HIP_CHECK(hipMemcpyAsync(h->host_word, dst, 4, hipMemcpyDeviceToHost, st));
         if (!h->count_event) GGET_HIP_CHECK(hipEventCreateWithFlags(&h->count_event, hipEventDisableTiming));
@@ -1450,12 +1481,13 @@
   h->pos_rows = h->pos_cur;
   if (h->varlen) {
     const Ws& w = h->ws;
-    if (int e = k_varlen_plan(ids, ldF, c.stacked_feat, h->pos_cur, h->wsp<int32_t>(w.key_len),
-                              c.kind == GGET_KIND_TASK ? h->wsp<int32_t>(w.pool_row) : nullptr, h->wsp<int32_t>(w.vl_cu),
-                              h->wsp<int64_t>(w.vl_ids), h->wsp<int64_t>(w.vl_pos), h->wsp<int32_t>(w.vl_rowb), h->wsp<int32_t>(w.vl_pad2c),
-                              h->wsp<int32_t>(w.vl_c2p), h->wsp<int32_t>(w.vl_status), B, S, h->tc, h->T, c.pad_token_id, st,
-                              h->wsp<int32_t>(w.vl_long)))
-      return e;
+    if (!h->plan_done)
+      if (int e = k_varlen_plan(ids, ldF, c.stacked_feat, h->pos_cur, h->wsp<int32_t>(w.key_len),
+                                c.kind == GGET_KIND_TASK ? h->wsp<int32_t>(w.pool_row) : nullptr, h->wsp<int32_t>(w.vl_cu),
+                                h->wsp<int64_t>(w.vl_ids), h->wsp<int64_t>(w.vl_pos), h->wsp<int32_t>(w.vl_rowb), h->wsp<int32_t>(w.vl_pad2c),
+                                h->wsp<int32_t>(w.vl_c2p), h->wsp<int32_t>(w.vl_status), B, S, h->tc, h->T, c.pad_token_id, st,
+                                h->wsp<int32_t>(w.vl_long)))
+        return e;
     h->ids = ids = h->wsp<int64_t>(w.vl_ids);
     ldF = c.stacked_feat;
     h->pos_rows = h->wsp<int64_t>(w.vl_pos);
@@ -1515,10 +1547,32 @@
                           h->wsp<int32_t>(w.row_idx), h->wsp<int32_t>(w.sel_src), h->wsp<int32_t>(w.sel_label), h->wsp<int32_t>(w.sel_tok),
                           h->wsp<int32_t>(w.hc_tot), sorted_head ? h->wsp<int32_t>(w.ss_state) : nullptr, s_);
   };
+  auto step_plan = [&](hipStream_t s_, int expect, int32_t* host_out, const int64_t* pos) -> int {
+    GgetStepPlan A;
+    memset(&A, 0, sizeof(A));
+    A.mask = attention_mask_dev; A.ids = input_ids_dev; A.pos = pos; A.labels = labels_dev;
+    A.ldF = c.stacked_feat; A.F = c.stacked_feat; A.B = B; A.S = S; A.n = n; A.pad_id = c.pad_token_id; A.expect = expect;
+    A.key_len = h->wsp<int32_t>(w.key_len); A.cu = h->wsp<int32_t>(w.vl_cu); A.row_b = h->wsp<int32_t>(w.vl_rowb);
+    A.pad2c = h->wsp<int32_t>(w.vl_pad2c); A.c2p = h->wsp<int32_t>(w.vl_c2p); A.long_list = h->wsp<int32_t>(w.vl_long);
+    A.ids_c = h->wsp<int64_t>(w.vl_ids); A.pos_c = h->wsp<int64_t>(w.vl_pos);
+    A.status = h->wsp<int32_t>(w.vl_status); A.count_out = A.status + 3; A.host_out = host_out;
+    A.cnt = h->wsp<int32_t>(w.cnt); A.m_off = h->wsp<int32_t>(w.m_off); A.l_off = h->wsp<int32_t>(w.l_off); A.counts = counts;
+    A.row_idx = h->wsp<int32_t>(w.row_idx); A.sel_src = h->wsp<int32_t>(w.sel_src); A.sel_label = h->wsp<int32_t>(w.sel_label);
+    A.sel_tok = h->wsp<int32_t>(w.sel_tok);
+    if (sorted_head) {
+      A.slot_state = h->wsp<int32_t>(w.ss_state); A.a_tok = h->wsp<int32_t>(w.ss_tok); A.a_cell = h->wsp<int32_t>(w.ss_cell);
+      A.c_l = h->wsp<int32_t>(w.ss_l); A.cellpos = h->wsp<int32_t>(w.ss_pos); A.tile_off = h->wsp<int32_t>(w.ss_tile);
+      A.total_p = h->wsp<int32_t>(w.ss_total); A.slot_elems = (long)d * d; A.tile_rows = head_tile_rows(d);
+    }
+    A.ws = h->wsp<int32_t>(w.sp_ws);
+    return k_step_plan(A, gget_gemm_num_cu() > 0 ? gget_gemm_num_cu() : 256, s_);
+  };
   h->presync_work = head_compact;
   h->presync_done = false;
+  if (!mask_is_3d && attention_mask_dev && (long)B * S * n < (1L << 31)) h->plan_work = step_plan;
   const int rc_bb = backbone_forward(h, tc_hint, input_ids_dev, c.stacked_feat, attention_mask_dev, position_ids_dev, B, S, st, mask_is_3d, labels_dev);
   h->presync_work = nullptr;
+  h->plan_work = nullptr;
   if (rc_bb) {
     if (sorted_head && h->presync_done)
       (void)hipMemsetAsync(h->wsp<int32_t>(w.ss_state), 0, 512, st);
@@ -1535,10 +1589,11 @@
     return e;
   h->head_sorted_fwd = false;
   if (sorted_head) {
-    if (int e = k_head_slot_sort(h->wsp<int32_t>(w.sel_src), h->wsp<int32_t>(w.row_idx), counts + 1, h->wsp<int32_t>(w.ss_state),
-                                 h->wsp<int32_t>(w.ss_tok), h->wsp<int32_t>(w.ss_cell), h->wsp<int32_t>(w.ss_l), h->wsp<int32_t>(w.ss_pos),
-                                 h->wsp<int32_t>(w.ss_tile), h->wsp<int32_t>(w.ss_total), T * n, n, (long)d * d, head_tile_rows(d), st))
-      return e;
+    if (!h->plan_done)
+      if (int e = k_head_slot_sort(h->wsp<int32_t>(w.sel_src), h->wsp<int32_t>(w.row_idx), counts + 1, h->wsp<int32_t>(w.ss_state),
+                                   h->wsp<int32_t>(w.ss_tok), h->wsp<int32_t>(w.ss_cell), h->wsp<int32_t>(w.ss_l), h->wsp<int32_t>(w.ss_pos),
+                                   h->wsp<int32_t>(w.ss_tile), h->wsp<int32_t>(w.ss_total), T * n, n, (long)d * d, head_tile_rows(d), st))
+        return e;
     GemmGroup g;
     memset(&g, 0, sizeof(g));
     g.count = 1;
@@ -2847,6 +2902,31 @@
   return k_head_slot_sort(sel_src, row_idx, lm_count, slot_state, a_tok, a_cell, c_l, cellpos, tile_off, total_p, cap, n, (long)slot_elems,
                           tile_rows, (hipStream_t)stream);
 }
+extern "C" uint64_t gget_op_step_plan_ws_bytes(int TP) { return TP > 0 ? (uint64_t)k_step_plan_ws_bytes(TP) : 0; }
+extern "C" int gget_op_step_plan(const int64_t* mask, const int64_t* ids, const int64_t* pos, const int64_t* labels, int ldF, int F, int B,
+                                 int S, int n, int pad_id, int expect, int32_t* key_len, int32_t* cu, int64_t* ids_c, int64_t* pos_c,
+                                 int32_t* row_b, int32_t* pad2c, int32_t* c2p, int32_t* long_list, int32_t* status, int32_t* cnt,
+                                 int32_t* m_off, int32_t* l_off, int32_t* counts, int32_t* row_idx, int32_t* sel_src, int32_t* sel_label,
+                                 int32_t* sel_tok, int32_t* slot_state, int32_t* a_tok, int32_t* a_cell, int32_t* c_l, int32_t* cellpos,
+                                 int32_t* tile_off, int32_t* total_p, int64_t slot_elems, int tile_rows, int32_t* ws, void* stream) {
+  GGET_REQUIRE(mask && ids && key_len && cu && ids_c && pos_c && row_b && pad2c && c2p && status && ws, "step_plan: null argument");
+  GGET_REQUIRE(cnt && m_off && l_off && counts && row_idx && sel_src && sel_label && sel_tok, "step_plan: null argument");
+  GGET_REQUIRE(!a_tok || (slot_state && a_cell && c_l && cellpos && tile_off && total_p && tile_rows > 0 && slot_elems >= 0 && n <= 32),
+               "step_plan: the slot sort needs all its arrays, tile_rows > 0 and n <= 32");
+  GGET_REQUIRE(B > 0 && S > 0 && F >= 1 && ldF >= F && n >= 1 && (long)B * S * n < (1L << 31), "step_plan: bad shape B %d S %d F %d ldF %d n %d",
+               B, S, F, ldF, n);
+  GgetStepPlan A;
+  memset(&A, 0, sizeof(A));
+  A.mask = mask; A.ids = ids; A.pos = pos; A.labels = labels;
+  A.ldF = ldF; A.F = F; A.B = B; A.S = S; A.n = n; A.pad_id = pad_id; A.expect = expect;
+  A.key_len = key_len; A.cu = cu; A.row_b = row_b; A.pad2c = pad2c; A.c2p = c2p; A.long_list = long_list; A.ids_c = ids_c; A.pos_c = pos_c;
+  A.status = status; A.count_out = status + 3;
+  A.cnt = cnt; A.m_off = m_off; A.l_off = l_off; A.counts = counts; A.row_idx = row_idx; A.sel_src = sel_src; A.sel_label = sel_label;
+  A.sel_tok = sel_tok;
+  A.slot_state = slot_state; A.a_tok = a_tok; A.a_cell = a_cell; A.c_l = c_l; A.cellpos = cellpos; A.tile_off = tile_off; A.total_p = total_p;
+  A.slot_elems = (long)slot_elems; A.tile_rows = tile_rows; A.ws = ws;
+  return k_step_plan(A, gget_gemm_num_cu() > 0 ? gget_gemm_num_cu() : 256, (hipStream_t)stream);
+}
 extern "C" int gget_op_head_cell_sum(const void* dxs, const int32_t* cellpos, const int32_t* cnt, const int32_t* l_off, const int32_t* pad2c,
                                      void* dhid, int TP, int d, int pad_row, void* stream) {
   GGET_REQUIRE(dxs && cellpos && cnt && l_off && dhid && TP > 0 && d > 0 && d % 8 == 0 && pad_row >= 0,
diff --git a/graph-gpt_amd/csrc/kernels.h b/graph-gpt_amd/csrc/kernels.h
--- a/graph-gpt_amd/csrc/kernels.h
+++ b/graph-gpt_amd/csrc/kernels.h
@@ -59,6 +59,22 @@
                    int32_t* row_idx, int32_t* sel_src, int32_t* sel_label, int32_t* sel_tok, int32_t* blk_tot, int32_t* slot_hist,
                    hipStream_t st);
 size_t k_head_compact_ws_bytes(int T);
+struct GgetStepPlan {
+  const int64_t *mask, *ids, *pos, *labels;
+  int ldF, F, B, S, n, pad_id;
+  int expect;
+  int32_t *key_len, *cu, *row_b, *pad2c, *c2p, *long_list;
+  int64_t *ids_c, *pos_c;
+  int32_t* status;
+  int32_t *count_out, *host_out;
+  int32_t *cnt, *m_off, *l_off, *counts, *row_idx, *sel_src, *sel_label, *sel_tok;
+  int32_t *slot_state, *a_tok, *a_cell, *c_l, *cellpos, *tile_off, *total_p;
+  long slot_elems;
+  int tile_rows;
+  int32_t* ws;
+};
+size_t k_step_plan_ws_bytes(int TP);
+int k_step_plan(const GgetStepPlan& A, int max_blocks, hipStream_t st);
 int k_gather_rows(const void* src, const int32_t* idx, const int32_t* count, void* dst, int cap, int d, int scatter,
                   hipStream_t st);
 int k_gather_rows_remap(const void* src, int32_t* idx, const int32_t* count, const int32_t* pad2c, void* dst, int cap, int d, int pad_row,
diff --git a/graph-gpt_amd/csrc/kernels.hip b/graph-gpt_amd/csrc/kernels.hip
--- a/graph-gpt_amd/csrc/kernels.hip
+++ b/graph-gpt_amd/csrc/kernels.hip
@@ -2646,16 +2646,16 @@
   return 0;
 }
 
-__global__ void __launch_bounds__(1024) varlen_scan_kernel(int32_t* __restrict__ key_len, int32_t* __restrict__ cu,
-                                                           int32_t* __restrict__ pool_row, int32_t* __restrict__ status, int B, int S,
-                                                           int expect_total, int32_t* __restrict__ long_list) {
-  __shared__ int wsum[16];
-  __shared__ int lsum[16];
+template <int NT>
+__device__ __forceinline__ void varlen_scan_block(int32_t* key_len, int32_t* cu, int32_t* pool_row, int32_t* status, int B, int S,
+                                                  int expect_total, int32_t* long_list) {
+  __shared__ int wsum[NT / 64];
+  __shared__ int lsum[NT / 64];
   __shared__ int carry_s, lcarry_s;
   const int tid = threadIdx.x, lane = tid & 63, wave = tid >> 6;
   if (tid == 0) { carry_s = 0; lcarry_s = 0; }
   __syncthreads();
-  for (int b0 = 0; b0 < B; b0 += 1024) {
+  for (int b0 = 0; b0 < B; b0 += NT) {
     const int b = b0 + tid;
     const int v = b < B ? key_len[b] : 0;
     int x = v;
@@ -2692,10 +2692,10 @@
       long_list[1 + 2 * B + lpos] = len;
     }
     __syncthreads();
-    if (tid == 1023) {
+    if (tid == NT - 1) {
       carry_s = base + x;
       int lt = lcarry_s;
-      for (int w = 0; w < 16; ++w) lt += lsum[w];
+      for (int w = 0; w < NT / 64; ++w) lt += lsum[w];
       lcarry_s = lt;
     }
     __syncthreads();
@@ -2707,12 +2707,14 @@
     if (carry_s != expect_total) status[2] = 1;
   }
 }
-__global__ void __launch_bounds__(kBlock) varlen_fill_kernel(const int64_t* __restrict__ ids, int ldF, int F, const int64_t* __restrict__ pos,
-                                                             const int32_t* __restrict__ key_len, const int32_t* __restrict__ cu,
-                                                             int64_t* __restrict__ ids_c, int64_t* __restrict__ pos_c,
-                                                             int32_t* __restrict__ row_b, int32_t* __restrict__ pad2c,
-                                                             int32_t* __restrict__ c2p, int B, int S, int tc, int t_rows, int64_t pad_id) {
-  const long i = (long)blockIdx.x * kBlock + threadIdx.x;
+__global__ void __launch_bounds__(1024) varlen_scan_kernel(int32_t* __restrict__ key_len, int32_t* __restrict__ cu,
+                                                           int32_t* __restrict__ pool_row, int32_t* __restrict__ status, int B, int S,
+                                                           int expect_total, int32_t* __restrict__ long_list) {
+  varlen_scan_block<1024>(key_len, cu, pool_row, status, B, S, expect_total, long_list);
+}
+__device__ __forceinline__ void varlen_fill_item(long i, const int64_t* ids, int ldF, int F, const int64_t* pos, const int32_t* key_len,
+                                                 const int32_t* cu, int64_t* ids_c, int64_t* pos_c, int32_t* row_b, int32_t* pad2c,
+                                                 int32_t* c2p, int B, int S, int tc, int t_rows, int64_t pad_id) {
   const long TP = (long)B * S;
   if (i < TP) {
     const int b = (int)(i / S), sq = (int)(i % S);
@@ -2734,6 +2736,14 @@
     c2p[r] = (int)i;
   }
 }
+__global__ void __launch_bounds__(kBlock) varlen_fill_kernel(const int64_t* __restrict__ ids, int ldF, int F, const int64_t* __restrict__ pos,
+                                                             const int32_t* __restrict__ key_len, const int32_t* __restrict__ cu,
+                                                             int64_t* __restrict__ ids_c, int64_t* __restrict__ pos_c,
+                                                             int32_t* __restrict__ row_b, int32_t* __restrict__ pad2c,
+                                                             int32_t* __restrict__ c2p, int B, int S, int tc, int t_rows, int64_t pad_id) {
+  varlen_fill_item((long)blockIdx.x * kBlock + threadIdx.x, ids, ldF, F, pos, key_len, cu, ids_c, pos_c, row_b, pad2c, c2p, B, S, tc,
+                   t_rows, pad_id);
+}
 __global__ void __launch_bounds__(1024) sum_lengths_kernel(const int32_t* __restrict__ key_len, int B, int32_t* __restrict__ out,
                                                            int32_t* __restrict__ host_out) {
   __shared__ int tot;
@@ -2854,6 +2864,224 @@
   return 0;
 }
 size_t k_head_compact_ws_bytes(int T) { return (size_t)((T + kBlock - 1) / kBlock) * 8; }
+
+constexpr int kPlanBlock = 256, kPlanWaves = kPlanBlock / 64;
+constexpr int kPlanSpins = 1 << 18;
+__global__ void __launch_bounds__(kPlanBlock) step_plan_kernel(GgetStepPlan A) {
+  __shared__ int sa[kPlanWaves], sb[kPlanWaves], sc[kPlanWaves], sd[kPlanWaves], hist[32], base_s[32], start[64], cells[64], bc[2];
+  const int tid = threadIdx.x, lane = tid & 63, wave = tid >> 6;
+  const int B = A.B, S = A.S, n = A.n, TP = B * S, NC = (TP + kPlanBlock - 1) / kPlanBlock;
+  int32_t* sync = A.ws;
+  int32_t* blk_tot = A.ws + 4;
+  int32_t* hist_ws = A.ws + 4 + 2 * NC;
+  const bool slots = A.a_tok != nullptr;
+  for (int b = blockIdx.x * kPlanWaves + wave; b < B; b += gridDim.x * kPlanWaves) {
+    int v = 0;
+    for (int s = lane; s < S; s += 64) v += A.mask[(size_t)b * S + s] != 0;
+    v = wave_sum_i32(v);
+    if (lane == 0) A.key_len[b] = v;
+  }
+  for (int vb = blockIdx.x; vb < NC; vb += gridDim.x) {
+    if (tid < 32) hist[tid] = 0;
+    __syncthreads();
+    const int t = vb * kPlanBlock + tid;
+    int c = 0;
+    if (t < TP) {
+      if (A.labels) {
+        for (int f = 0; f < n; ++f)
+          if (A.labels[(size_t)t * n + f] != -100) {
+            ++c;
+            if (slots) atomicAdd(&hist[f], 1);
+          }
+      } else {
+        c = n;
+      }
+      A.cnt[t] = c;
+    }
+    const int wm = wave_sum_i32(c > 0), wl = wave_sum_i32(c);
+    if (lane == 0) { sa[wave] = wm; sb[wave] = wl; }
+    __syncthreads();
+    if (tid == 0) {
+      int m = 0, l = 0;
+      for (int w = 0; w < kPlanWaves; ++w) { m += sa[w]; l += sb[w]; }
+      blk_tot[2 * vb] = m;
+      blk_tot[2 * vb + 1] = l;
+    }
+    if (slots && tid < 32) hist_ws[vb * 32 + tid] = A.labels ? hist[tid] : (tid < n ? min(kPlanBlock, TP - vb * kPlanBlock) : 0);
+    __syncthreads();
+  }
+  asm volatile("s_waitcnt vmcnt(0)" ::: "memory");
+  __syncthreads();
+  if (tid == 0) {
+    __builtin_amdgcn_fence(__ATOMIC_RELEASE, "agent");
+    asm volatile("s_waitcnt vmcnt(0)" ::: "memory");
+    const int ticket = __hip_atomic_fetch_add(&sync[0], 1, __ATOMIC_RELAXED, __HIP_MEMORY_SCOPE_AGENT);
+    bc[0] = ticket == (int)gridDim.x - 1;
+    if (bc[0]) {
+      __builtin_amdgcn_fence(__ATOMIC_ACQUIRE, "agent");
+      asm volatile("s_waitcnt vmcnt(0)" ::: "memory");
+    }
+  }
+  __syncthreads();
+  if (bc[0]) {
+    int v = 0;
+    for (int b = tid; b < B; b += kPlanBlock) v += A.key_len[b];
+    v = wave_sum_i32(v);
+    if (lane == 0) sa[wave] = v;
+    __syncthreads();
+    int total = 0;
+    for (int w = 0; w < kPlanWaves; ++w) total += sa[w];
+    const int tc = A.expect > 0 ? A.expect : total;
+    if (tid == 0) {
+      *A.count_out = total;
+      if (A.host_out) __hip_atomic_store(A.host_out, total, __ATOMIC_RELEASE, __HIP_MEMORY_SCOPE_SYSTEM);
+    }
+    if (tc > 0 && (tc + 63) / 64 * 64 < TP) varlen_scan_block<kPlanBlock>(A.key_len, A.cu, nullptr, A.status, B, S, tc, A.long_list);
+    asm volatile("s_waitcnt vmcnt(0)" ::: "memory");
+    __syncthreads();
+    if (tid == 0) {
+      __builtin_amdgcn_fence(__ATOMIC_RELEASE, "agent");
+      asm volatile("s_waitcnt vmcnt(0)" ::: "memory");
+      __hip_atomic_store(&sync[1], tc + 1, __ATOMIC_RELAXED, __HIP_MEMORY_SCOPE_AGENT);
+      bc[1] = tc + 1;
+    }
+  } else if (tid == 0) {
+    int flag = 0;
+    for (int spin = 0; spin < kPlanSpins; ++spin) {
+      flag = __hip_atomic_load(&sync[1], __ATOMIC_RELAXED, __HIP_MEMORY_SCOPE_AGENT);
+      if (flag) break;
+      __builtin_amdgcn_s_sleep(8);
+    }
+    if (flag) {
+      __builtin_amdgcn_fence(__ATOMIC_ACQUIRE, "agent");
+      asm volatile("s_waitcnt vmcnt(0)" ::: "memory");
+    } else {
+      A.status[5] = 1;
+    }
+    bc[1] = flag;
+  }
+  __syncthreads();
+  if (bc[1]) {
+    const int tc = bc[1] - 1, t_rows = (tc + 63) / 64 * 64;
+    const bool vl = tc > 0 && t_rows < TP;
+    const int pad_row = t_rows > tc ? tc : 0;
+    if (vl) {
+      const long nfill = (long)TP + (t_rows - tc);
+      const int fb = (int)((blockIdx.x + gridDim.x / 2) % gridDim.x);
+      for (long i = (long)fb * kPlanBlock + tid; i < nfill; i += (long)gridDim.x * kPlanBlock)
+        varlen_fill_item(i, A.ids, A.ldF, A.F, A.pos, A.key_len, A.cu, A.ids_c, A.pos_c, A.row_b, A.pad2c, A.c2p, B, S, tc, t_rows,
+                         (int64_t)A.pad_id);
+    }
+    if (slots) {
+      if (tid < 64) {
+        int cf = 0;
+        if (lane < n)
+          for (int j = 0; j < NC; ++j) cf += hist_ws[j * 32 + lane];
+        const int pc = (cf + A.tile_rows - 1) / A.tile_rows * A.tile_rows;
+        int inc = pc;
+#pragma unroll
+        for (int o = 1; o < 64; o <<= 1) {
+          const int y = __shfl_up(inc, o, 64);
+          if (lane >= o) inc += y;
+        }
+        cells[lane] = cf;
+        start[lane] = inc - pc;
+      }
+      __syncthreads();
+      if (blockIdx.x == gridDim.x - 1) {
+        if (tid == 0) *A.total_p = start[n];
+        if (tid <= n) A.slot_state[2 * n + tid] = start[tid];
+        for (int f = 0; f < n; ++f) {
+          const int lo = start[f] + cells[f], hi = start[f + 1];
+          for (int p = lo + tid; p < hi; p += kPlanBlock) { A.a_tok[p] = 0; A.a_cell[p] = 0; A.c_l[p] = -1; }
+          for (int t = start[f] / A.tile_rows + tid; t < start[f + 1] / A.tile_rows; t += kPlanBlock)
+            A.tile_off[t] = (int32_t)((long)f * A.slot_elems);
+        }
+      }
+    }
+    for (int vb = blockIdx.x; vb < NC; vb += gridDim.x) {
+      if (slots && tid < 32) {
+        int bs = 0;
+        if (tid < n) {
+          bs = start[tid];
+          for (int j = 0; j < vb; ++j) bs += hist_ws[j * 32 + tid];
+        }
+        base_s[tid] = bs;
+        hist[tid] = 0;
+      }
+      int pm = 0, pl = 0;
+      for (int j = tid; j < vb; j += kPlanBlock) { pm += blk_tot[2 * j]; pl += blk_tot[2 * j + 1]; }
+      pm = wave_sum_i32(pm);
+      pl = wave_sum_i32(pl);
+      const int t = vb * kPlanBlock + tid;
+      const int c = t < TP ? A.cnt[t] : 0;
+      int im = c > 0, il = c;
+#pragma unroll
+      for (int o = 1; o < 64; o <<= 1) {
+        const int am = __shfl_up(im, o, 64), al = __shfl_up(il, o, 64);
+        if (lane >= o) { im += am; il += al; }
+      }
+      if (lane == 63) { sa[wave] = im; sb[wave] = il; }
+      if (lane == 0) { sc[wave] = pm; sd[wave] = pl; }
+      __syncthreads();
+      int bm = 0, bl = 0;
+      for (int w = 0; w < kPlanWaves; ++w) { bm += sc[w]; bl += sd[w]; }
+      for (int w = 0; w < wave; ++w) { bm += sa[w]; bl += sb[w]; }
+      if (vb == NC - 1 && tid == kPlanBlock - 1) { A.counts[0] = bm + im; A.counts[1] = bl + il; }
+      if (t < TP) {
+        const int m = bm + im - (c > 0);
+        int j = bl + il - c;
+        A.m_off[t] = m;
+        A.l_off[t] = j;
+        if (c > 0) {
+          A.row_idx[m] = t;
+          int arow = t;
+          if (slots && vl) {
+            const int b = t / S, sq = t % S;
+            arow = sq < A.key_len[b] ? A.cu[b] + sq : pad_row;
+          }
+          for (int f = 0; f < n; ++f) {
+            const int64_t lab = A.labels ? A.labels[(size_t)t * n + f] : 0;
+            if (!A.labels || lab != -100) {
+              A.sel_src[j] = m * n + f;
+              A.sel_label[j] = (int32_t)lab;
+              A.sel_tok[j] = t;
+              if (slots) {
+                const int p = base_s[f] + atomicAdd(&hist[f], 1);
+                A.a_tok[p] = arow;
+                A.a_cell[p] = m * n + f;
+                A.c_l[p] = j;
+                A.cellpos[j] = p;
+              }
+              ++j;
+            }
+          }
+        }
+      }
+      __syncthreads();
+    }
+  }
+  __syncthreads();
+  if (tid == 0) {
+    if (__hip_atomic_fetch_add(&sync[2], 1, __ATOMIC_RELAXED, __HIP_MEMORY_SCOPE_AGENT) == (int)gridDim.x - 1) {
+      __hip_atomic_store(&sync[0], 0, __ATOMIC_RELAXED, __HIP_MEMORY_SCOPE_AGENT);
+      __hip_atomic_store(&sync[1], 0, __ATOMIC_RELAXED, __HIP_MEMORY_SCOPE_AGENT);
+      __hip_atomic_store(&sync[2], 0, __ATOMIC_RELAXED, __HIP_MEMORY_SCOPE_AGENT);
+    }
+  }
+}
+size_t k_step_plan_ws_bytes(int TP) { return (size_t)(4 + 34 * ((TP + kPlanBlock - 1) / kPlanBlock)) * 4; }
+int k_step_plan(const GgetStepPlan& A, int max_blocks, hipStream_t st) {
+  if (A.a_tok && A.n > 32) { gget_set_error("step plan: next_n_token %d > 32 with the slot-sorted head", A.n); return 2; }
+  const long TP = (long)A.B * A.S;
+  long g = (TP + 63 + kPlanBlock - 1) / kPlanBlock;
+  if (g < (A.B + kPlanWaves - 1) / kPlanWaves) g = (A.B + kPlanWaves - 1) / kPlanWaves;
+  if (g > max_blocks) g = max_blocks;
+  if (g < 1) g = 1;
+  hipLaunchKernelGGL(step_plan_kernel, dim3((unsigned)g), dim3(kPlanBlock), 0, st, A);
+  GGET_LAUNCH_CHECK();
+  return 0;
+}
 
 int k_gather_rows(const void* src, const int32_t* idx, const int32_t* count, void* dst, int cap, int d, int scatter,
                   hipStream_t st) {
diff --git a/graph-gpt_amd/csrc/menu.h b/graph-gpt_amd/csrc/menu.h
--- a/graph-gpt_amd/csrc/menu.h
+++ b/graph-gpt_amd/csrc/menu.h
@@ -32,6 +32,7 @@
   int ls_norm_bwd_wide;
   int no_varlen;
   int count_copy;
+  int step_plan;
   int embed_sorted;
   int occupy_fat;
   int deterministic;
@@ -99,6 +100,7 @@
     {&LaunchMenu::no_ls_norm_fusion, 0, "GGET_NO_LS_NORM_FUSION", true, 0, "set: LayerScale residual and the next RMSNorm as separate launches"},
     {&LaunchMenu::no_varlen, 0, "GGET_NO_VARLEN", true, 0, "set: the padded token grid instead of the var-len layout"},
     {&LaunchMenu::count_copy, 0, "GGET_COUNT_COPY", false, 0, "1: token count back by device-to-host copy + event instead of a polled host word"},
+    {&LaunchMenu::step_plan, 21, "GGET_STEP_PLAN", false, 1, "0: key lengths, token count, head compaction, var-len plan and slot sort as seven launches instead of one"},
     {&LaunchMenu::embed_sorted, 20, "GGET_EMBED_SORTED", true, 0, "set: embedding backward always as the sorted scatter-add"},
     {&LaunchMenu::rms_rows, 0, "GGET_RMS_ROWS", false, 4, "RMSNorm backward rows per wave"},
     {&LaunchMenu::ce_generic, 19, "GGET_CE_GENERIC", true, 0, "set: cross-entropy never on the vectorised row kernels"},
diff --git a/include/gget.h b/include/gget.h
--- a/include/gget.h
+++ b/include/gget.h
@@ -340,6 +340,13 @@
 int gget_op_head_slot_sort(const int32_t* sel_src, const int32_t* row_idx, const int32_t* lm_count, int32_t* slot_state, int32_t* a_tok,
                            int32_t* a_cell, int32_t* c_l, int32_t* cellpos, int32_t* tile_off, int32_t* total_p, int cap, int n,
                            int64_t slot_elems, int tile_rows, void* stream);
+uint64_t gget_op_step_plan_ws_bytes(int TP);
+int gget_op_step_plan(const int64_t* mask, const int64_t* ids, const int64_t* pos, const int64_t* labels, int ldF, int F, int B, int S, int n,
+                      int pad_id, int expect, int32_t* key_len, int32_t* cu, int64_t* ids_c, int64_t* pos_c, int32_t* row_b, int32_t* pad2c,
+                      int32_t* c2p, int32_t* long_list, int32_t* status, int32_t* cnt, int32_t* m_off, int32_t* l_off, int32_t* counts,
+                      int32_t* row_idx, int32_t* sel_src, int32_t* sel_label, int32_t* sel_tok, int32_t* slot_state, int32_t* a_tok,
+                      int32_t* a_cell, int32_t* c_l, int32_t* cellpos, int32_t* tile_off, int32_t* total_p, int64_t slot_elems, int tile_rows,
+                      int32_t* ws, void* stream);
 int gget_op_head_cell_sum(const void* dxs, const int32_t* cellpos, const int32_t* cnt, const int32_t* l_off, const int32_t* pad2c,
                           void* dhid, int TP, int d, int pad_row, void* stream);
 int gget_op_gather_rows(const void* src, const int32_t* idx, const int32_t* count, void* dst, int cap, int d, int scatter, void* stream);
```

Measured after the change: 822,100 graph-tokens/s, median of 6. About the same (+0.3%).
